# qqaazz0222/DuCoSy-GAN

Hardware: AMD Instinct MI355X
Metric: CycleGAN train-step images/sec at 512x512 bs=8/GPU (higher is better)
Workload: dtype f32 via f16x3 MFMA (power-of-two scaled hi/lo fp16 split, 22 significant bits, three products; f32 accumulation and storage); 1 GPU; full soft-tissue CycleGAN train step: 2x Generator (ResNet-9 + CBAM) + 2x PatchGAN, 9 G loss terms + 2 D losses, 3 Adam steps; img_size=512, per_gpu_batch=8, global_batch=8, residual_blocks=9, input_channels=3, parallelism=dp1

## Files before the change

ducosy-gan_amd/csrc/cbam.hip:

```cpp
#include "common.hpp"

constexpr int SERIAL_UNROLL = 8;

namespace dcs {

__global__ __launch_bounds__(256) void ca_forward_kernel(const float* __restrict__ ymax, const float* __restrict__ sc,
                                                         const float* __restrict__ sh, const float* __restrict__ w1,
                                                         const float* __restrict__ w2, int C, int Cr,
                                                         float* __restrict__ ca) {
    extern __shared__ float sm[];
    float* vmax = sm;
    float* h = sm + C;
    float* h0 = h + Cr;
    const int n = blockIdx.x, tid = threadIdx.x;
    for (int c = tid; c < C; c += blockDim.x) vmax[c] = fmaf(ymax[n * C + c], sc[n * C + c], sh[n * C + c]);
    __syncthreads();
    for (int j = tid; j < Cr; j += blockDim.x) {
        float a = 0.f;
        for (int c = 0; c < C; ++c) a = fmaf(w1[j * C + c], vmax[c], a);
        h[j] = a > 0.f ? a : 0.f;
        h0[j] = 0.f;
    }
    __syncthreads();
    for (int c = tid; c < C; c += blockDim.x) {
// ... 254 lines not shown
        v[k] = reinterpret_cast<const float4*>(y + (p0 + k) * 256)[lane];
        d[k] = reinterpret_cast<const float4*>(dout + (p0 + k) * 256)[lane];
    }
#pragma unroll
    for (int k = 0; k < PX; ++k) {
        float acc = 0.f;
        acc = fmaf(d[k].x, fmaf(v[k].x, s.x, b.x) * a.x, acc);
        acc = fmaf(d[k].y, fmaf(v[k].y, s.y, b.y) * a.y, acc);
        acc = fmaf(d[k].z, fmaf(v[k].z, s.z, b.z) * a.z, acc);
        acc = fmaf(d[k].w, fmaf(v[k].w, s.w, b.w) * a.w, acc);
        acc = wave_sum(acc);
        if (lane == 0) {
            const float g = sa[p0 + k];
            dpre[p0 + k] = acc * g * (1.f - g);
        }
    }
}

template <int PX>
__global__ __launch_bounds__(256) void cb_bwd_dsa_sums_kernel(const float* __restrict__ dout, const float* __restrict__ y,
                                                              const float* __restrict__ sc, const float* __restrict__ sh,
                                                              const float* __restrict__ ca, const float* __restrict__ sa,
                                                              int HW, int nchunk, float* __restrict__ dpre,
                                                              Sum2* __restrict__ p1) {
    __shared__ float4 s_a[256], s_b[256];
    const int n = blockIdx.x, chunk = blockIdx.y, tid = threadIdx.x;
    const int lane = tid & 63, plane = tid >> 6;
    const int p_per = (HW + nchunk - 1) / nchunk;
    const int p0 = chunk * p_per;
    const int pend = min(HW, p0 + p_per);
    const float4 s = reinterpret_cast<const float4*>(sc + (long long)n * 256)[lane];
    const float4 b = reinterpret_cast<const float4*>(sh + (long long)n * 256)[lane];
    const float4 a = reinterpret_cast<const float4*>(ca + (long long)n * 256)[lane];
    float4 A = make_float4(0.f, 0.f, 0.f, 0.f), B = A;
    const long long base = (long long)n * HW;
    for (int p = p0 + plane; p < pend; p += 4 * PX) {
        float4 v[PX], d[PX];
        float gg[PX];
#pragma unroll
        for (int k = 0; k < PX; ++k) {
            const int pk = p + 4 * k < pend ? p + 4 * k : pend - 1;
            v[k] = reinterpret_cast<const float4*>(y + (base + pk) * 256)[lane];
            d[k] = reinterpret_cast<const float4*>(dout + (base + pk) * 256)[lane];
            gg[k] = sa[base + pk];
        }
#pragma unroll
        for (int k = 0; k < PX; ++k) {
            const bool ok = p + 4 * k < pend;
            const float zx = fmaf(v[k].x, s.x, b.x), zy = fmaf(v[k].y, s.y, b.y);
            const float zz = fmaf(v[k].z, s.z, b.z), zw = fmaf(v[k].w, s.w, b.w);
            float acc = 0.f;
            acc = fmaf(d[k].x, zx * a.x, acc);
            acc = fmaf(d[k].y, zy * a.y, acc);
            acc = fmaf(d[k].z, zz * a.z, acc);
            acc = fmaf(d[k].w, zw * a.w, acc);
            acc = wave_sum(acc);
            if (ok) {
                if (lane == 0) dpre[base + p + 4 * k] = acc * gg[k] * (1.f - gg[k]);
                const float g = gg[k];
                const float dx = d[k].x * g, dy_ = d[k].y * g, dz = d[k].z * g, dw = d[k].w * g;
                A.x = fmaf(dx, zx, A.x); A.y = fmaf(dy_, zy, A.y); A.z = fmaf(dz, zz, A.z); A.w = fmaf(dw, zw, A.w);
                B.x += dx; B.y += dy_; B.z += dz; B.w += dw;
            }
        }
    }
    s_a[tid] = A;
    s_b[tid] = B;
    __syncthreads();
    if (plane == 0) {
#pragma unroll
        for (int l = 1; l < 4; ++l) {
            const float4 u = s_a[l * 64 + lane], w = s_b[l * 64 + lane];
            A.x += u.x; A.y += u.y; A.z += u.z; A.w += u.w;
            B.x += w.x; B.y += w.y; B.z += w.z; B.w += w.w;
        }
        Sum2* o = p1 + ((long long)n * nchunk + chunk) * 256 + 4 * lane;
        o[0] = Sum2{A.x, B.x};
        o[1] = Sum2{A.y, B.y};
        o[2] = Sum2{A.z, B.z};
        o[3] = Sum2{A.w, B.w};
    }
}

__global__ void cb_bwd_dsin_kernel(const float* __restrict__ dpre, const float* __restrict__ wsa, int H, int W, int ksa,
                                   long long P, float* __restrict__ dsin) {
    const long long q = (long long)blockIdx.x * blockDim.x + threadIdx.x;
    if (q >= P) return;
    const int HW = H * W;
    const int n = (int)(q / HW);
    const int rem = (int)(q - (long long)n * HW);
    const int qy = rem / W, qx = rem - qy * W;
    const int r = ksa / 2, taps = ksa * ksa;
    float a0 = 0.f, a1 = 0.f;
    for (int ty = 0; ty < ksa; ++ty) {
        int yy = qy - ty + r;
        if (yy < 0 || yy >= H) continue;
        for (int tx = 0; tx < ksa; ++tx) {
            int xx = qx - tx + r;
            if (xx < 0 || xx >= W) continue;
            float d = dpre[(long long)n * HW + yy * W + xx];
            a0 = fmaf(wsa[ty * ksa + tx], d, a0);
            a1 = fmaf(wsa[taps + ty * ksa + tx], d, a1);
        }
    }
    dsin[q * 2 + 0] = a0;
    dsin[q * 2 + 1] = a1;
}

__global__ __launch_bounds__(256) void cb_bwd_dwsa_partial_kernel(const float* __restrict__ dpre,
                                                                  const float* __restrict__ sin_, int H, int W,
                                                                  int ksa, long long P, int nchunk,
                                                                  float* __restrict__ part) {
    __shared__ float red[4];
    const int t = blockIdx.x, chunk = blockIdx.y;
    const int taps = ksa * ksa, r = ksa / 2;
    const int ch = t / taps, tt = t - ch * taps;
    const int ty = tt / ksa, tx = tt - ty * ksa;
    const int per = (int)((P + nchunk - 1) / nchunk);
    const int p0 = chunk * per, p1 = (int)min(P, (long long)p0 + per);
    const int HW = H * W;
    float acc = 0.f;
#pragma unroll 4
    for (int p = p0 + threadIdx.x; p < p1; p += blockDim.x) {
        const int n = p / HW;
        const int rem = p - n * HW;
        const int py = rem / W, px = rem - py * W;
        const int yy = py + ty - r, xx = px + tx - r;
        if (yy >= 0 && yy < H && xx >= 0 && xx < W)
            acc = fmaf(dpre[p], sin_[(n * HW + yy * W + xx) * 2 + ch], acc);
    }
    acc = block_sum_256(acc, red);
    if (threadIdx.x == 0) part[(long long)chunk * gridDim.x + t] = acc;
}

__global__ void cb_bwd_dwsa_final_kernel(const float* __restrict__ part, int nt, int nchunk, float* __restrict__ dwsa) {
    int t = blockIdx.x * blockDim.x + threadIdx.x;
    if (t >= nt) return;
    double s = 0.0;
#pragma unroll SERIAL_UNROLL
    for (int k = 0; k < nchunk; ++k) s += part[(long long)k * nt + t];
    dwsa[t] = (float)s;
}

struct Sum3 {
    float a, b, c;
};

__global__ __launch_bounds__(256) void cb_bwd_sums_kernel(const float* __restrict__ dout, const float* __restrict__ y,
                                                          const float* __restrict__ sc, const float* __restrict__ sh,
                                                          const float* __restrict__ ca, const float* __restrict__ sa,
                                                          const float* __restrict__ dsin,
                                                          const int* __restrict__ sarg, int HW, int C, int nchunk,
                                                          Sum3* __restrict__ parts) {
    const int n = blockIdx.x, chunk = blockIdx.y, tid = threadIdx.x;
    const int p_per = (HW + nchunk - 1) / nchunk;
    const int p0 = chunk * p_per;
    const int p1 = min(HW, p0 + p_per);
    const bool packed = (C <= 256) && (256 % C == 0);
    const int lanes = packed ? 256 / C : 1;
    const int plane = packed ? tid / C : 0;
    __shared__ float s_a[256], s_b[256], s_c[256];
    const float invC = 1.f / (float)C;
    for (int cbase = 0; cbase < C; cbase += (packed ? C : 256)) {
        const int c = packed ? (tid % C) : (cbase + tid);
        float A = 0.f, B = 0.f, Cc = 0.f;
        if (c < C) {
            const long long nc = (long long)n * C + c;
            const float s = sc[nc], b = sh[nc], a = ca[nc];
            for (int p = p0 + plane; p < p1; p += lanes) {
                const long long pp = (long long)n * HW + p;
                const long long o = pp * C + c;
                float z = fmaf(y[o], s, b);
                float dzc = fmaf(dout[o], sa[pp], dsin[pp * 2] * invC);
                if (sarg[pp] == c) dzc += dsin[pp * 2 + 1];
                float dz0 = dzc * a;
                A = fmaf(dzc, z, A);
                B += dz0;
                Cc = fmaf(dz0, z, Cc);
            }
        }
        if (packed) {
            s_a[tid] = A; s_b[tid] = B; s_c[tid] = Cc;
            __syncthreads();
            if (plane == 0) {
                for (int l = 1; l < lanes; ++l) { A += s_a[l * C + c]; B += s_b[l * C + c]; Cc += s_c[l * C + c]; }
                parts[((long long)n * nchunk + chunk) * C + c] = Sum3{A, B, Cc};
            }
            __syncthreads();
        } else if (c < C) {
            parts[((long long)n * nchunk + chunk) * C + c] = Sum3{A, B, Cc};
        }
    }
}

template <bool HALF>
__global__ __launch_bounds__(256) void cb_bwd_sums4_kernel(const float* __restrict__ dout, const float* __restrict__ y,
                                                           const float* __restrict__ sc, const float* __restrict__ sh,
                                                           const float* __restrict__ ca, const float* __restrict__ sa,
                                                           const float* __restrict__ dsin,
                                                           const int* __restrict__ sarg, int HW, int C, int nchunk,
                                                           Sum3* __restrict__ parts, const Sum2* __restrict__ p1) {
    __shared__ float4 s_a[256], s_b[256], s_c[256];
    const int n = blockIdx.x, chunk = blockIdx.y, tid = threadIdx.x;
    const int C4 = C >> 2, lanes = 256 / C4;
    const int c4 = tid % C4, plane = tid / C4;
    const int p_per = (HW + nchunk - 1) / nchunk;
    const int p0 = chunk * p_per;
    const int pend = min(HW, p0 + p_per);
    const int nc = n * C + 4 * c4;
    const float4 s = *reinterpret_cast<const float4*>(sc + nc);
    const float4 b = *reinterpret_cast<const float4*>(sh + nc);
    const float4 a = *reinterpret_cast<const float4*>(ca + nc);
    const float invC = 1.f / (float)C;
    float4 A = make_float4(0.f, 0.f, 0.f, 0.f), B = A, Cc = A;
    for (int p = p0 + plane; p < pend; p += lanes) {
        const long long pp = (long long)n * HW + p;
        const float4 yv = reinterpret_cast<const float4*>(y + pp * C)[c4];
        const float2 ds = reinterpret_cast<const float2*>(dsin)[pp];
        const int am = sarg[pp] - 4 * c4;
        const float d0 = ds.x * invC;
        float z, dzc, dz0;
        if constexpr (HALF) {
#define DCS_SUMS_LANE(X, K)                                   \
        z = fmaf(yv.X, s.X, b.X);                             \
        dzc = d0;                                             \
        if (am == K) dzc += ds.y;                             \
        A.X = fmaf(dzc, z, A.X);                              \
        B.X += dzc;
            DCS_SUMS_LANE(x, 0)
            DCS_SUMS_LANE(y, 1)
            DCS_SUMS_LANE(z, 2)
            DCS_SUMS_LANE(w, 3)
#undef DCS_SUMS_LANE
        } else {
            const float4 dv = reinterpret_cast<const float4*>(dout + pp * C)[c4];
            const float g = sa[pp];
#define DCS_SUMS_LANE(X, K)                                   \
        z = fmaf(yv.X, s.X, b.X);                             \
        dzc = fmaf(dv.X, g, d0);                              \
        if (am == K) dzc += ds.y;                             \
        dz0 = dzc * a.X;                                      \
        A.X = fmaf(dzc, z, A.X);                              \
        B.X += dz0;                                           \
        Cc.X = fmaf(dz0, z, Cc.X);
            DCS_SUMS_LANE(x, 0)
            DCS_SUMS_LANE(y, 1)
            DCS_SUMS_LANE(z, 2)
            DCS_SUMS_LANE(w, 3)
#undef DCS_SUMS_LANE
        }
    }
    s_a[tid] = A; s_b[tid] = B; s_c[tid] = Cc;
    __syncthreads();
    if (plane == 0) {
        for (int l = 1; l < lanes; ++l) {
            const float4 u = s_a[l * C4 + c4], v = s_b[l * C4 + c4], w = s_c[l * C4 + c4];
            A.x += u.x; A.y += u.y; A.z += u.z; A.w += u.w;
            B.x += v.x; B.y += v.y; B.z += v.z; B.w += v.w;
            Cc.x += w.x; Cc.y += w.y; Cc.z += w.z; Cc.w += w.w;
        }
        Sum3* o = parts + ((long long)n * nchunk + chunk) * C + 4 * c4;
        if constexpr (HALF) {
            const Sum2* q = p1 + ((long long)n * nchunk + chunk) * C + 4 * c4;
            const float ax = A.x + q[0].a, ay = A.y + q[1].a, az = A.z + q[2].a, aw = A.w + q[3].a;
            o[0] = Sum3{ax, a.x * (B.x + q[0].b), a.x * ax};
            o[1] = Sum3{ay, a.y * (B.y + q[1].b), a.y * ay};
            o[2] = Sum3{az, a.z * (B.z + q[2].b), a.z * az};
            o[3] = Sum3{aw, a.w * (B.w + q[3].b), a.w * aw};
        } else {
            o[0] = Sum3{A.x, B.x, Cc.x};
            o[1] = Sum3{A.y, B.y, Cc.y};
            o[2] = Sum3{A.z, B.z, Cc.z};
            o[3] = Sum3{A.w, B.w, Cc.w};
        }
    }
}

__global__ __launch_bounds__(256) void cb_bwd_ca_kernel(const Sum3* __restrict__ parts, int nchunk,
                                                        const float* __restrict__ ymax, const float* __restrict__ sc,
                                                        const float* __restrict__ sh, const float* __restrict__ ca,
                                                        const float* __restrict__ w1, const float* __restrict__ w2,
                                                        int HW, int C, int Cr, Sum3* __restrict__ coef,
                                                        float* __restrict__ dwpart) {
    extern __shared__ float sm[];
    float* vmax = sm;
    float* dpc = vmax + C;
    float* hp = dpc + C;
    float* dhm = hp + Cr;
    float* S1 = dhm + Cr;
    float* S2 = S1 + C;
    __shared__ float red[2][4];
    const int tid = threadIdx.x, n = blockIdx.x;
    for (int c = tid; c < C; c += blockDim.x) {
        const long long nc = (long long)n * C + c;
        double A = 0.0, B = 0.0, Cc = 0.0;
#pragma unroll SERIAL_UNROLL
        for (int k = 0; k < nchunk; ++k) {
            Sum3 p = parts[((long long)n * nchunk + k) * C + c];
            A += p.a; B += p.b; Cc += p.c;
        }
        vmax[c] = fmaf(ymax[nc], sc[nc], sh[nc]);
        float g = ca[nc];
        dpc[c] = (float)A * g * (1.f - g);
        S1[c] = (float)B;
        S2[c] = (float)Cc;
    }
    __syncthreads();
    for (int j = 0; j < Cr; ++j) {
        float a = 0.f, b = 0.f;
        for (int c = tid; c < C; c += blockDim.x) {
            a = fmaf(w1[j * C + c], vmax[c], a);
            b = fmaf(w2[c * Cr + j], dpc[c], b);
        }
        a = wave_sum(a);
        b = wave_sum(b);
        if ((tid & 63) == 0) { red[0][tid >> 6] = a; red[1][tid >> 6] = b; }
        __syncthreads();
        if (tid == 0) {
            float hpre = red[0][0] + red[0][1] + red[0][2] + red[0][3];
            float dh = red[1][0] + red[1][1] + red[1][2] + red[1][3];
            hp[j] = hpre;
            dhm[j] = hpre > 0.f ? dh : 0.f;
        }
        __syncthreads();
    }
    float* dw1 = dwpart + (long long)n * 2 * C * Cr;
    float* dw2 = dw1 + (long long)C * Cr;
    const float inv = 1.f / (float)HW;
    for (int c = tid; c < C; c += blockDim.x) {
        float dvm = 0.f;
        for (int j = 0; j < Cr; ++j) {
            dvm = fmaf(w1[j * C + c], dhm[j], dvm);
            dw2[c * Cr + j] = dpc[c] * (hp[j] > 0.f ? hp[j] : 0.f);
            dw1[j * C + c] = dhm[j] * vmax[c];
        }
        coef[(long long)n * C + c] = Sum3{(S1[c] + dvm) * inv, (S2[c] + dvm * vmax[c]) * inv, dvm};
    }
}

__global__ void cb_bwd_dw_reduce_kernel(const float* __restrict__ dwpart, int N, int CCr, float* __restrict__ dw1,
                                        float* __restrict__ dw2) {
    int i = blockIdx.x * blockDim.x + threadIdx.x;
    if (i >= 2 * CCr) return;
    float s = 0.f;
#pragma unroll SERIAL_UNROLL
    for (int n = 0; n < N; ++n) s += dwpart[(long long)n * 2 * CCr + i];
    if (i < CCr) dw1[i] = s;
    else dw2[i - CCr] = s;
}

__global__ void cb_bwd_apply_kernel(const float* __restrict__ dout, const float* __restrict__ y,
                                    const float* __restrict__ sc, const float* __restrict__ sh,
                                    const float* __restrict__ ca, const float* __restrict__ sa,
                                    const float* __restrict__ dsin, const int* __restrict__ sarg,
                                    const int* __restrict__ yarg, const Sum3* __restrict__ coef, int HW, int C,
                                    long long total, float* __restrict__ dy, float* __restrict__ rng) {
    const long long i0 = (long long)blockIdx.x * blockDim.x + threadIdx.x;
    const bool live = i0 < total;
    const long long i = live ? i0 : total - 1;
    const int c = (int)(i % C);
    const long long pp = i / C;
    const int n = (int)(pp / HW);
    const int p = (int)(pp - (long long)n * HW);
    const long long nc = (long long)n * C + c;
    const float s = sc[nc], b = sh[nc];
    const float z = fmaf(y[i], s, b);
    float dzc = fmaf(dout[i], sa[pp], dsin[pp * 2] * (1.f / (float)C));
    if (sarg[pp] == c) dzc += dsin[pp * 2 + 1];
    const Sum3 k = coef[nc];
    float dz = dzc * ca[nc];
    if (yarg[nc] == p) dz += k.c;
    const float v = s * (dz - k.a - z * k.b);
    if (live) dy[i] = v;
    range_note(rng, fabsf(v));
}

__global__ __launch_bounds__(256) void cb_bwd_apply4_kernel(const float* __restrict__ dout, const float* __restrict__ y,
                                                            const float* __restrict__ sc, const float* __restrict__ sh,
                                                            const float* __restrict__ ca, const float* __restrict__ sa,
                                                            const float* __restrict__ dsin, const int* __restrict__ sarg,
                                                            const int* __restrict__ yarg, const Sum3* __restrict__ coef,
                                                            int HW, int C, int total4, float* __restrict__ dy,
                                                            float* __restrict__ rng) {
    const int i40 = blockIdx.x * blockDim.x + threadIdx.x;
    const bool live = i40 < total4;
    const int i4 = live ? i40 : total4 - 1;
    const int C4 = C >> 2;
    const int pp = i4 / C4;
    const int c4 = i4 - pp * C4;
    const int n = pp / HW;
    const int p = pp - n * HW;
    const int nc = n * C + 4 * c4;
    const float4 s = *reinterpret_cast<const float4*>(sc + nc);
    const float4 b = *reinterpret_cast<const float4*>(sh + nc);
    const float4 a = *reinterpret_cast<const float4*>(ca + nc);
    const int4 ya = *reinterpret_cast<const int4*>(yarg + nc);
    const float4 k0 = *reinterpret_cast<const float4*>(reinterpret_cast<const float*>(coef + nc));
    const float4 k1 = *reinterpret_cast<const float4*>(reinterpret_cast<const float*>(coef + nc) + 4);
    const float4 k2 = *reinterpret_cast<const float4*>(reinterpret_cast<const float*>(coef + nc) + 8);
    const float4 yv = reinterpret_cast<const float4*>(y)[i4];
    const float4 dv = reinterpret_cast<const float4*>(dout)[i4];
    const float g = sa[pp];
    const float2 ds = reinterpret_cast<const float2*>(dsin)[pp];
    const int am = sarg[pp] - 4 * c4;
    const float d0 = ds.x * (1.f / (float)C);
    float4 o;
#define DCS_APPLY_LANE(X, K, KA, KB, KC)                      \
    {                                                         \
        const float z = fmaf(yv.X, s.X, b.X);                 \
        float dzc = fmaf(dv.X, g, d0);                        \
        if (am == K) dzc += ds.y;                             \
        float dz = dzc * a.X;                                 \
        if (ya.X == p) dz += KC;                              \
        o.X = s.X * (dz - KA - z * KB);                       \
    }
    DCS_APPLY_LANE(x, 0, k0.x, k0.y, k0.z)
    DCS_APPLY_LANE(y, 1, k0.w, k1.x, k1.y)
    DCS_APPLY_LANE(z, 2, k1.z, k1.w, k2.x)
    DCS_APPLY_LANE(w, 3, k2.y, k2.z, k2.w)
#undef DCS_APPLY_LANE
    if (live) reinterpret_cast<float4*>(dy)[i4] = o;
    range_note(rng, absmax4(o));
}

template <int PX>
__global__ __launch_bounds__(256) void cb_bwd_apply4x_kernel(const float* __restrict__ dout, const float* __restrict__ y,
                                                             const float* __restrict__ sc, const float* __restrict__ sh,
                                                             const float* __restrict__ ca, const float* __restrict__ sa,
                                                             const float* __restrict__ dsin, const int* __restrict__ sarg,
                                                             const int* __restrict__ yarg, const Sum3* __restrict__ coef,
                                                             int HW, int C, float* __restrict__ dy, float* __restrict__ rng) {
    const int C4 = C >> 2;
    const int ppb = 256 / C4;
    const int c4 = threadIdx.x % C4, pl = threadIdx.x / C4;
    const int pp0 = blockIdx.x * ppb * PX;
    const int n = pp0 / HW;
    const int nc = n * C + 4 * c4;
    const float4 s = *reinterpret_cast<const float4*>(sc + nc);
    const float4 b = *reinterpret_cast<const float4*>(sh + nc);
    const float4 a = *reinterpret_cast<const float4*>(ca + nc);
    const int4 ya = *reinterpret_cast<const int4*>(yarg + nc);
    const float4 k0 = *reinterpret_cast<const float4*>(reinterpret_cast<const float*>(coef + nc));
    const float4 k1 = *reinterpret_cast<const float4*>(reinterpret_cast<const float*>(coef + nc) + 4);
    const float4 k2 = *reinterpret_cast<const float4*>(reinterpret_cast<const float*>(coef + nc) + 8);
    const float rC = 1.f / (float)C;
    float m = 0.f;
#pragma unroll
    for (int k = 0; k < PX; ++k) {
        const int pp = pp0 + k * ppb + pl;
        const int p = pp - n * HW;
        const int i4 = pp * C4 + c4;
        const float4 yv = reinterpret_cast<const float4*>(y)[i4];
        const float4 dv = reinterpret_cast<const float4*>(dout)[i4];
        const float g = sa[pp];
        const float2 ds = reinterpret_cast<const float2*>(dsin)[pp];
        const int am = sarg[pp] - 4 * c4;
        const float d0 = ds.x * rC;
        float4 o;
#define DCS_APPLY_LANE(X, K, KA, KB, KC)                      \
    {                                                         \
        const float z = fmaf(yv.X, s.X, b.X);                 \
        float dzc = fmaf(dv.X, g, d0);                        \
        if (am == K) dzc += ds.y;                             \
        float dz = dzc * a.X;                                 \
        if (ya.X == p) dz += KC;                              \
        o.X = s.X * (dz - KA - z * KB);                       \
    }
        DCS_APPLY_LANE(x, 0, k0.x, k0.y, k0.z)
        DCS_APPLY_LANE(y, 1, k0.w, k1.x, k1.y)
        DCS_APPLY_LANE(z, 2, k1.z, k1.w, k2.x)
        DCS_APPLY_LANE(w, 3, k2.y, k2.z, k2.w)
#undef DCS_APPLY_LANE
        reinterpret_cast<float4*>(dy)[i4] = o;
        m = fmaxf(m, absmax4(o));
    }
    range_note(rng, m);
}

static inline int cb_chunks(int N, int HW) {
    int want = (int)cdiv(1024, N);
    int maxc = (int)cdiv(HW, 64);
    int c = want < maxc ? want : maxc;
    return c < 1 ? 1 : c;
}
static inline int sa_wchunks(long long P) {
    long long c = cdiv(P, 4096);
    if (c < 1) c = 1;
    if (c > 64) c = 64;
    return (int)c;
}

struct CbWs {
    float* dpre;
    float* dsin;
    float* wpart;
    Sum3* parts;
    Sum2* p1;
    Sum3* coef;
    float* dwpart;
    size_t total;
};
static CbWs cb_layout(void* base, int N, int H, int W, int C, int Cr, int ksa) {
    CbWs w;
    long long P = (long long)N * H * W;
    size_t off = 0;
    char* b = reinterpret_cast<char*>(base);
    w.dpre = reinterpret_cast<float*>(b + off); off = align_up(off + P * sizeof(float), 256);
    w.dsin = reinterpret_cast<float*>(b + off); off = align_up(off + 2 * P * sizeof(float), 256);
    w.wpart = reinterpret_cast<float*>(b + off); off = align_up(off + (size_t)sa_wchunks(P) * 2 * ksa * ksa * sizeof(float), 256);
    int nch = cb_chunks(N, H * W);
    w.parts = reinterpret_cast<Sum3*>(b + off); off = align_up(off + (size_t)N * nch * C * sizeof(Sum3), 256);
    w.p1 = reinterpret_cast<Sum2*>(b + off); off = align_up(off + (size_t)N * nch * C * sizeof(Sum2), 256);
    w.coef = reinterpret_cast<Sum3*>(b + off); off = align_up(off + (size_t)N * C * sizeof(Sum3), 256);
    w.dwpart = reinterpret_cast<float*>(b + off); off = align_up(off + (size_t)N * 2 * C * Cr * sizeof(float), 256);
    w.total = off;
    return w;
}

}

using namespace dcs;

extern "C" int dcs_cbam_forward(const float* x, const float* y, const float* scale, const float* shift,
                                const float* ymax, const float* w1, const float* w2, const float* wsa, int N, int H,
                                int W, int C, int Cr, int ksa, float* ca, float* sin_, int32_t* sarg, float* sa,
                                float* out, float* rng, void* stream) {
    if (!x || !y || !scale || !shift || !ymax || !w1 || !w2 || !wsa || !ca || !sin_ || !sarg || !sa || !out)
        return fail(DCS_E_INVALID, "cbam_forward: null pointer");
    if (N <= 0 || H <= 0 || W <= 0 || C <= 0 || C % 4 != 0 || Cr <= 0 || ksa <= 0 || (ksa & 1) == 0)
        return fail(DCS_E_INVALID, "cbam_forward: bad dims");
    hipStream_t s = as_stream(stream);
    long long P = (long long)N * H * W;
    hipLaunchKernelGGL(ca_forward_kernel, dim3(N), dim3(256), (size_t)(C + 2 * Cr) * sizeof(float), s, ymax, scale,
                       shift, w1, w2, C, Cr, ca);
    int e = check_launch("ca_forward");
    if (e) return e;
    const int nq = cb_nq(C);
#define DCS_CB16(K, NQ, ...) hipLaunchKernelGGL((K<NQ>), dim3(cb16_blocks(P)), dim3(256), 0, s, __VA_ARGS__)
    if (nq == 4) DCS_CB16(sa_reduce16_kernel, 4, y, scale, shift, ca, H * W, C, P, sin_, sarg);
    else if (nq == 2) DCS_CB16(sa_reduce16_kernel, 2, y, scale, shift, ca, H * W, C, P, sin_, sarg);
    else if (nq == 1) DCS_CB16(sa_reduce16_kernel, 1, y, scale, shift, ca, H * W, C, P, sin_, sarg);
    else hipLaunchKernelGGL(sa_reduce_kernel, dim3((unsigned)cdiv(P, 4)), dim3(256), 0, s, y, scale, shift, ca, H * W, C,
                            P, sin_, sarg);
    e = check_launch("sa_reduce");
    if (e) return e;
    if ((e = range_zero(rng, s))) return e;
    if (nq == 4) DCS_CB16(sa_apply16_kernel, 4, x, y, scale, shift, ca, sin_, wsa, H, W, C, ksa, P, sa, out, rng);
    else if (nq == 2) DCS_CB16(sa_apply16_kernel, 2, x, y, scale, shift, ca, sin_, wsa, H, W, C, ksa, P, sa, out, rng);
    else if (nq == 1) DCS_CB16(sa_apply16_kernel, 1, x, y, scale, shift, ca, sin_, wsa, H, W, C, ksa, P, sa, out, rng);
    else hipLaunchKernelGGL(sa_apply_kernel, dim3((unsigned)cdiv(P, 4)), dim3(256), 0, s, x, y, scale, shift, ca, sin_,
                            wsa, H, W, C, ksa, P, sa, out, rng);
    return check_launch("sa_apply");
}

extern "C" size_t dcs_cbam_backward_workspace_size(int N, int H, int W, int C, int Cr, int ksa) {
    if (N <= 0 || H <= 0 || W <= 0 || C <= 0 || Cr <= 0 || ksa <= 0) return 0;
    return cb_layout(nullptr, N, H, W, C, Cr, ksa).total;
}

extern "C" int dcs_cbam_backward(const float* dout, const float* y, const float* scale, const float* shift,
                                 const float* ymax, const int32_t* yargmax, const float* w1, const float* w2,
                                 const float* wsa, const float* ca, const float* sin_, const int32_t* sarg,
                                 const float* sa, int N, int H, int W, int C, int Cr, int ksa, float* dy, float* dw1,
                                 float* dw2, float* dwsa, void* ws, size_t ws_bytes, float* rng, void* stream) {
    if (!dout || !y || !scale || !shift || !ymax || !yargmax || !w1 || !w2 || !wsa || !ca || !sin_ || !sarg || !sa ||
        !dy || !dw1 || !dw2 || !dwsa || !ws)
        return fail(DCS_E_INVALID, "cbam_backward: null pointer");
    if (N <= 0 || H <= 0 || W <= 0 || C <= 0 || C % 4 != 0 || Cr <= 0 || ksa <= 0)
        return fail(DCS_E_INVALID, "cbam_backward: bad dims");
    if (ws_bytes < dcs_cbam_backward_workspace_size(N, H, W, C, Cr, ksa))
        return fail(DCS_E_WORKSPACE, "cbam_backward: workspace too small");
    if ((long long)N * H * W * 2 >= (1LL << 31))
        return fail(DCS_E_INVALID, "cbam_backward: N*H*W*2 must fit in 31 bits");
    CbWs w = cb_layout(ws, N, H, W, C, Cr, ksa);
    hipStream_t s = as_stream(stream);
    const long long P = (long long)N * H * W;
    const int HW = H * W;
    constexpr int DPX = 4;
    const int nch = cb_chunks(N, HW);
    const bool fused = C == 256;
    if (fused)
        hipLaunchKernelGGL(cb_bwd_dsa_sums_kernel<DPX>, dim3(N, nch), dim3(256), 0, s, dout, y, scale, shift, ca, sa, HW,
                           nch, w.dpre, w.p1);
    else if (C == 256 && HW % DPX == 0)
        hipLaunchKernelGGL(cb_bwd_dsa64x_kernel<DPX>, dim3((unsigned)cdiv(P, 4 * DPX)), dim3(256), 0, s, dout, y, scale,
                           shift, ca, sa, HW, P, w.dpre);
    else
        hipLaunchKernelGGL(cb_bwd_dsa_kernel, dim3((unsigned)cdiv(P, 4)), dim3(256), 0, s, dout, y, scale, shift, ca, sa,
                           HW, C, P, w.dpre);
    int e = check_launch("cb_bwd_dsa");
    if (e) return e;
    hipLaunchKernelGGL(cb_bwd_dsin_kernel, dim3((unsigned)cdiv(P, 256)), dim3(256), 0, s, w.dpre, wsa, H, W, ksa, P,
                       w.dsin);
    if ((e = check_launch("cb_bwd_dsin"))) return e;
    const int nt = 2 * ksa * ksa, nwc = sa_wchunks(P);
    hipLaunchKernelGGL(cb_bwd_dwsa_partial_kernel, dim3(nt, nwc), dim3(256), 0, s, w.dpre, sin_, H, W, ksa, P, nwc,
                       w.wpart);
    if ((e = check_launch("cb_bwd_dwsa_partial"))) return e;
    hipLaunchKernelGGL(cb_bwd_dwsa_final_kernel, dim3((unsigned)cdiv(nt, 128)), dim3(128), 0, s, w.wpart, nt, nwc, dwsa);
    if ((e = check_launch("cb_bwd_dwsa_final"))) return e;
    const bool v4 = (C % 4 == 0) && (C / 4 <= 256) && (256 % (C / 4) == 0);
    if (fused)
        hipLaunchKernelGGL(cb_bwd_sums4_kernel<true>, dim3(N, nch), dim3(256), 0, s, dout, y, scale, shift, ca, sa, w.dsin,
                           sarg, HW, C, nch, w.parts, w.p1);
    else if (v4)
        hipLaunchKernelGGL(cb_bwd_sums4_kernel<false>, dim3(N, nch), dim3(256), 0, s, dout, y, scale, shift, ca, sa, w.dsin,
                           sarg, HW, C, nch, w.parts, nullptr);
    else
        hipLaunchKernelGGL(cb_bwd_sums_kernel, dim3(N, nch), dim3(256), 0, s, dout, y, scale, shift, ca, sa, w.dsin,
                           sarg, HW, C, nch, w.parts);
    if ((e = check_launch("cb_bwd_sums"))) return e;
    hipLaunchKernelGGL(cb_bwd_ca_kernel, dim3(N), dim3(256), (size_t)(4 * C + 2 * Cr) * sizeof(float), s, w.parts, nch,
                       ymax, scale, shift, ca, w1, w2, HW, C, Cr, w.coef, w.dwpart);
    if ((e = check_launch("cb_bwd_ca"))) return e;
    hipLaunchKernelGGL(cb_bwd_dw_reduce_kernel, dim3((unsigned)cdiv(2LL * C * Cr, 256)), dim3(256), 0, s, w.dwpart, N,
                       C * Cr, dw1, dw2);
    if ((e = check_launch("cb_bwd_dw_reduce"))) return e;
    if ((e = range_zero(rng, s))) return e;
    const long long total = P * C;
    const int C4 = C / 4;
    constexpr int APX = 4;
    if (total / 4 < (1LL << 31) && (long long)N * C < (1LL << 31) && C4 <= 256 && 256 % C4 == 0 &&
        HW % (APX * (256 / C4)) == 0) {
        hipLaunchKernelGGL(cb_bwd_apply4x_kernel<APX>, dim3((unsigned)(P / (APX * (256 / C4)))), dim3(256), 0, s, dout,
                           y, scale, shift, ca, sa, w.dsin, sarg, yargmax, w.coef, HW, C, dy, rng);
    } else if (total / 4 < (1LL << 31) && (long long)N * C < (1LL << 31)) {
        const int total4 = (int)(total / 4);
        hipLaunchKernelGGL(cb_bwd_apply4_kernel, dim3((unsigned)cdiv(total4, 256)), dim3(256), 0, s, dout, y, scale,
                           shift, ca, sa, w.dsin, sarg, yargmax, w.coef, HW, C, total4, dy, rng);
    } else {
        hipLaunchKernelGGL(cb_bwd_apply_kernel, dim3((unsigned)cdiv(total, 256)), dim3(256), 0, s, dout, y, scale, shift,
                           ca, sa, w.dsin, sarg, yargmax, w.coef, HW, C, total, dy, rng);
    }
    return check_launch("cb_bwd_apply");
}
#undef DCS_CB16
```

ducosy-gan_amd/csrc/conv.hip:

```cpp
#include "common.hpp"
#include "conv_common.hpp"

namespace dcs {

typedef __bf16 bf16x8 __attribute__((ext_vector_type(8)));

constexpr int MMA_F32 = 0, MMA_BF16 = 1, MMA_BF16X3 = 3, MMA_BF16X6 = 6;
constexpr int MMA_BF16P = 2;
constexpr int MMA_F16X3 = 7;
constexpr int MMA_F16 = 8;

template <int MMA>
constexpr int lde_bf16() { return MMA == MMA_BF16X3 ? 72 : 40; }

typedef unsigned int u32x4v __attribute__((ext_vector_type(4)));
template <int MMA>
__device__ __forceinline__ void split8(const float4& a, const float4& b, bf16x8& hi, bf16x8& lo) {
    const floatx8 f = {a.x, a.y, a.z, a.w, b.x, b.y, b.z, b.w};
    hi = __builtin_convertvector(f, bf16x8);
    if constexpr (MMA == MMA_BF16X3) {
        u32x4v w;
        __builtin_memcpy(&w, &hi, 16);
        floatx8 r;
#pragma unroll
// ... 1789 lines not shown
    for (int p = 0; p < ny; ++p)
        for (int q = 0; q < nx; ++q) {
            const int yp = ay[p], xp = ax[q];
            if (yp >= 1 && yp <= H && xp >= 1 && xp <= W) continue;
            const int ri = yp == 0 ? xp : (yp == Hp - 1 ? Wp + xp : 2 * Wp + 2 * (yp - 1) + (xp == 0 ? 0 : 1));
            for (int q = 0; q < nsplit; ++q) {
                const float4 v = reinterpret_cast<const float4*>(ring)[(((long long)q * N + n) * ringlen + ri) * C4 + c4];
                s.x += v.x; s.y += v.y; s.z += v.z; s.w += v.w;
            }
        }
    *o = s;
}

__global__ void upsample2_grad_kernel(const float* __restrict__ du, float* __restrict__ dx, int N, int H,
                                      int W, int C4) {
    long long idx = (long long)blockIdx.x * blockDim.x + threadIdx.x;
    long long total = (long long)N * H * W * C4;
    if (idx >= total) return;
    int c4 = (int)(idx % C4);
    long long t = idx / C4;
    int j = (int)(t % W); t /= W;
    int i = (int)(t % H);
    int n = (int)(t / H);
    const float4* u = reinterpret_cast<const float4*>(du);
    const long long W2 = 2LL * W;
    long long b = (((long long)n * 2 * H + 2 * i) * W2 + 2 * j) * C4 + c4;
    float4 a0 = u[b], a1 = u[b + C4], a2 = u[b + W2 * C4], a3 = u[b + W2 * C4 + C4];
    reinterpret_cast<float4*>(dx)[idx] =
        make_float4(a0.x + a1.x + a2.x + a3.x, a0.y + a1.y + a2.y + a3.y, a0.z + a1.z + a2.z + a3.z,
                    a0.w + a1.w + a2.w + a3.w);
}

static int validate(const dcs_conv_desc* d, bool rows) {
    if (!d) return fail(DCS_E_INVALID, "null descriptor");
    if (d->N <= 0 || d->Hs <= 0 || d->Ws <= 0 || d->Cs <= 0 || d->Ho <= 0 || d->Wo <= 0 || d->Co <= 0)
        return fail(DCS_E_INVALID, "conv: non-positive dimension");
    if (d->KH <= 0 || d->KW <= 0 || d->KH * d->KW > 64) return fail(DCS_E_INVALID, "conv: bad kernel");
    if (d->up != 1 && d->up != 2) return fail(DCS_E_INVALID, "conv: up must be 1 or 2");
    if (d->stride != 1 && d->stride != 2) return fail(DCS_E_INVALID, "conv: stride must be 1 or 2");
    if (d->parity < 0 || d->parity > 2) return fail(DCS_E_INVALID, "conv: parity must be 0, 1 or 2");
    if (d->parity == 1 && (d->stride != 2 || d->up != 1 || d->pad_mode != DCS_PAD_ZERO))
        return fail(DCS_E_INVALID, "conv: parity rows need stride 2, no upsample, zero pad");
    if (d->parity == 2 && (d->stride != 1 || d->up != 1 || d->pad_mode != DCS_PAD_ZERO || d->KH != 3 ||
                           d->KW != 3 || d->Ho != 2 * d->Hs || d->Wo != 2 * d->Ws))
        return fail(DCS_E_INVALID, "conv: sub-pixel rows describe nearest-x2 + 3x3 zero-pad conv (up=1, Ho=2Hs)");
    if (d->pad_mode == DCS_PAD_REFLECT && (d->pt >= d->Hs * d->up || d->pl >= d->Ws * d->up))
        return fail(DCS_E_INVALID, "conv: reflect pad larger than the input");
    if (d->csplit < 0 || d->csplit > d->Cs) return fail(DCS_E_INVALID, "conv: bad csplit");
    if (d->cw < 0 || d->cw > d->Cs) return fail(DCS_E_INVALID, "conv: bad cw (weight channels)");
    if (d->mma != MMA_F32 && d->mma != MMA_BF16 && d->mma != MMA_BF16X3 && d->mma != MMA_BF16X6 && d->mma != MMA_F16X3 &&
        d->mma != MMA_F16)
        return fail(DCS_E_INVALID, "conv: mma must be DCS_MMA_F32, DCS_MMA_BF16, DCS_MMA_BF16X3, DCS_MMA_BF16X6, DCS_MMA_F16X3 or DCS_MMA_F16");
    if ((d->mma == MMA_F16X3 || d->mma == MMA_F16) && (!d->rng_a || !d->rng_b || d->rng_a_n <= 0 || d->rng_b_n <= 0 ||
                                d->rng_a_n > 1024 || d->rng_b_n > 1024))
        return fail(DCS_E_INVALID, "conv: DCS_MMA_F16X3 / DCS_MMA_F16 need the operand range records rng_a / rng_b (1..1024 partial maxima)");
    if (!d->parity) {
        int Hv = d->Hs * d->up, Wv = d->Ws * d->up;
        (void)Hv; (void)Wv;
    }
    (void)rows;
    return DCS_OK;
}

static bool vec4_ok(const dcs_conv_desc* d, const float* src) {
    const long long extent = (long long)(d->N - 1) * d->s_n + (long long)(d->Hs - 1) * d->s_h +
                             (long long)(d->Ws - 1) * d->s_w + d->Cs;
    return d->Cs == 4 && d->s_c == 1 && d->csplit == 4 && (d->s_w % 4 == 0) && (d->s_h % 4 == 0) &&
           (d->s_n % 4 == 0) && ((reinterpret_cast<uintptr_t>(src) & 15) == 0) && d->s_n >= 0 && d->s_h >= 0 &&
           d->s_w >= 0 && extent * 4 < (long long)OOB_OFF - 64;
}

static bool vec_ok(const dcs_conv_desc* d, const float* src) {
    const long long extent = (long long)(d->N - 1) * d->s_n + (long long)(d->Hs - 1) * d->s_h +
                             (long long)(d->Ws - 1) * d->s_w + d->Cs;
    return (d->Cs % 16 == 0) && d->s_c == 1 && d->csplit == d->Cs &&
           (d->s_w % 4 == 0) && (d->s_h % 4 == 0) && (d->s_n % 4 == 0) &&
           ((reinterpret_cast<uintptr_t>(src) & 15) == 0) && extent * 4 < (long long)OOB_OFF - 64 &&
           d->s_n >= 0 && d->s_h >= 0 && d->s_w >= 0;
}

bool narrow_tiled_ok(const dcs_conv_desc& d, const float* src);
int launch_narrow_rows_tiled(const dcs_conv_desc& d, const float* src, const float* wp, const float* bias,
                             const float* psc, const float* psh, float* out, hipStream_t s);
bool narrow_small_ok(const dcs_conv_desc& d, const float* src);
int launch_narrow_rows_small(const dcs_conv_desc& d, const float* src, const float* wp, const float* bias,
                             const float* psc, const float* psh, float* out, hipStream_t s);
bool narrow_wgrad_tiled_ok(const dcs_conv_desc& d, const float* src);
int narrow_wgrad_tiled_blocks(const dcs_conv_desc& d);
int launch_narrow_wgrad_tiled(const dcs_conv_desc& d, const float* dy, const float* src, const float* psc,
                              const float* psh, float* part, hipStream_t s);

}

using namespace dcs;

extern "C" int dcs_pack_weights_r(const float* w, int Cout, int Cin, int KH, int KW, int kind, int ci_count,
                                  int Kpad, int ncols, int nmajor, float* out, float* rng, void* stream);
namespace {
unsigned pack_blocks(long long total) {
    const long long b = cdiv(total, 256);
    return (unsigned)(b < 1 ? 1 : (b > DCS_RANGE_PARTS ? DCS_RANGE_PARTS : b));
}
}
extern "C" int dcs_pack_weights(const float* w, int Cout, int Cin, int KH, int KW, int kind, int ci_count,
                                int Kpad, int ncols, int nmajor, float* out, void* stream) {
    return dcs_pack_weights_r(w, Cout, Cin, KH, KW, kind, ci_count, Kpad, ncols, nmajor, out, nullptr, stream);
}

namespace {
const char* pack_args_error(const float* w, int Cout, int Cin, int KH, int KW, int kind, int ci_count, int Kpad,
                            int ncols, const float* out) {
    if (!w || !out || Cout <= 0 || Cin <= 0 || KH <= 0 || KW <= 0 || Kpad <= 0 || ncols <= 0 || ci_count <= 0 ||
        (kind != 5 && ci_count > Cin) || (kind == 5 && ci_count < Cin) || kind < 0 ||
        (kind & 7) > 5 || (kind & ~(7 | DCS_PACK_KSLICE)) ||
        ((kind & DCS_PACK_KSLICE) && (((kind & 7) != 0 && (kind & 7) != 1) ||
                                      ((kind & 7) == 0 ? Cin : Cout) % 16 != 0)))
        return "pack_weights: bad arguments";
    if ((kind == 3 || kind == 4) && (KH != 3 || KW != 3)) return "pack_weights: sub-pixel kinds need 3x3";
    return nullptr;
}
}

extern "C" int dcs_pack_weights_r(const float* w, int Cout, int Cin, int KH, int KW, int kind, int ci_count,
                                  int Kpad, int ncols, int nmajor, float* out, float* rng, void* stream) {
    if (const char* err = pack_args_error(w, Cout, Cin, KH, KW, kind, ci_count, Kpad, ncols, out))
        return fail(DCS_E_INVALID, err);
    long long total = (long long)Kpad * ncols;
    if (rng)
        hipLaunchKernelGGL(pack_weights_r_kernel, dim3(pack_blocks(total)), dim3(256), 0, as_stream(stream), w, Cout, Cin,
                           KH, KW, kind, ci_count, Kpad, ncols, nmajor, out, rng);
    else
        hipLaunchKernelGGL(pack_weights_kernel, dim3((unsigned)cdiv(total, 256)), dim3(256), 0, as_stream(stream), w,
                           Cout, Cin, KH, KW, kind, ci_count, Kpad, ncols, nmajor, out);
    return check_launch("pack_weights");
}

namespace dcs {
__global__ __launch_bounds__(256) void pack_split_h3_kernel(const float* __restrict__ wp, long long total, int ldb,
                                                            const float* __restrict__ rng, int rng_n,
                                                            _Float16* __restrict__ out) {
    const float sc = __builtin_ldexpf(1.f, f16x3_exp(rng, rng_n));
    for (long long i = (long long)blockIdx.x * 256 + threadIdx.x; i < total; i += (long long)gridDim.x * 256) {
        const long long r = i / ldb, k = i - r * ldb;
        const float v = wp[i] * sc;
        const _Float16 h = (_Float16)v;
        out[2 * r * ldb + k] = h;
        out[(2 * r + 1) * ldb + k] = (_Float16)(v - (float)h);
    }
}
}

extern "C" int dcs_pack_split_h3(const float* wpack, int rows, int ldb, const float* rng, int rng_n, void* out,
                                 void* stream) {
    if (!wpack || !rng || !out || rows <= 0 || ldb <= 0 || rng_n <= 0) return fail(DCS_E_INVALID, "pack_split_h3: bad arguments");
    const long long total = (long long)rows * ldb;
    const long long blocks = cdiv(total, 256) < 1024 ? cdiv(total, 256) : 1024;
    hipLaunchKernelGGL(pack_split_h3_kernel, dim3((unsigned)blocks), dim3(256), 0, as_stream(stream), wpack, total, ldb,
                       rng, rng_n, reinterpret_cast<_Float16*>(out));
    return check_launch("pack_split_h3");
}

namespace dcs {
namespace {
__device__ __forceinline__ int pack_job_of(const dcs_pack_job* __restrict__ jobs, int njobs, int b, bool second) {
    int lo = 0, hi = njobs - 1;
    while (lo < hi) {
        const int mid = (lo + hi + 1) >> 1;
// ... 806 lines not shown
        const long long total = (long long)d.Co * d.KH * d.KW * d.Cs;
        hipLaunchKernelGGL(wgrad_reduce_kernel, dim3((unsigned)cdiv(total, 256)), dim3(256), 0, s, w, ns, d.Co, d.Cs,
                           d.KH, d.KW, d.Cs, dw);
        return check_launch("conv_wgrad_reduce");
    }
    const bool res = d.Cs == 256 && d.KH == 3 && d.KW == 3 && d.up == 1 && d.stride == 1 && !d.parity &&
                     d.pro_act == DCS_ACT_NONE && d.epi_act == DCS_ACT_NONE;
    const bool v4 = !vec && vec4_ok(dp, x) && d.pro_act == DCS_ACT_NONE && !d.parity;
    const bool dy_small = (long long)d.N * d.Ho * d.Wo * d.Co * 4 < (long long)OOB_OFF - 64;
    if ((d.mma == MMA_F16X3 || d.mma == MMA_F16) && v4 && d.Cs == 4 && !d.parity && dy_small &&
               d.pro_act == DCS_ACT_NONE && (p.BM == 128 || d.Co == 64) && class_geom(d, 0).Mx >= 16) {
        const bool plain = d.pad_mode == DCS_PAD_ZERO && d.up == 1;
        if (d.mma == MMA_F16X3) {
            if (plain) hipLaunchKernelGGL((conv_wgrad_x6_kernel<2, MMA_F16X3, true>), grid, dim3(NT), 0, s, d, dy, x, psc, psh, w, 2 * p.kt_per_split, gn, gm);
            else hipLaunchKernelGGL((conv_wgrad_x6_kernel<0, MMA_F16X3, true>), grid, dim3(NT), 0, s, d, dy, x, psc, psh, w, 2 * p.kt_per_split, gn, gm);
        } else {
            if (plain) hipLaunchKernelGGL((conv_wgrad_x6_kernel<2, MMA_F16, true>), grid, dim3(NT), 0, s, d, dy, x, psc, psh, w, 2 * p.kt_per_split, gn, gm);
            else hipLaunchKernelGGL((conv_wgrad_x6_kernel<0, MMA_F16, true>), grid, dim3(NT), 0, s, d, dy, x, psc, psh, w, 2 * p.kt_per_split, gn, gm);
        }
    } else if (d.mma != MMA_F32 && vec && dy_small && (p.BM == 128 || (d.Co == 64 && (d.mma == MMA_F16X3 || d.mma == MMA_F16))) &&
               d.parity != 1 && class_geom(d, 0).Mx >= 16) {
        const bool plain = d.pro_act == DCS_ACT_NONE && d.pad_mode == DCS_PAD_ZERO && d.up == 1;
        const bool lrelu = d.pro_act == DCS_ACT_LRELU && d.pad_mode == DCS_PAD_ZERO && d.up == 1;
        if (d.mma == MMA_F16X3) {
            if (res) hipLaunchKernelGGL((conv_wgrad_x6_kernel<1, MMA_F16X3>), grid, dim3(NT), 0, s, d, dy, x, psc, psh, w, 2 * p.kt_per_split, gn, gm);
            else if (plain) hipLaunchKernelGGL((conv_wgrad_x6_kernel<2, MMA_F16X3>), grid, dim3(NT), 0, s, d, dy, x, psc, psh, w, 2 * p.kt_per_split, gn, gm);
            else if (lrelu) hipLaunchKernelGGL((conv_wgrad_x6_kernel<3, MMA_F16X3>), grid, dim3(NT), 0, s, d, dy, x, psc, psh, w, 2 * p.kt_per_split, gn, gm);
            else hipLaunchKernelGGL((conv_wgrad_x6_kernel<0, MMA_F16X3>), grid, dim3(NT), 0, s, d, dy, x, psc, psh, w, 2 * p.kt_per_split, gn, gm);
        } else if (d.mma == MMA_F16) {
            if (res) hipLaunchKernelGGL((conv_wgrad_x6_kernel<1, MMA_F16>), grid, dim3(NT), 0, s, d, dy, x, psc, psh, w, 2 * p.kt_per_split, gn, gm);
            else if (plain) hipLaunchKernelGGL((conv_wgrad_x6_kernel<2, MMA_F16>), grid, dim3(NT), 0, s, d, dy, x, psc, psh, w, 2 * p.kt_per_split, gn, gm);
            else if (lrelu) hipLaunchKernelGGL((conv_wgrad_x6_kernel<3, MMA_F16>), grid, dim3(NT), 0, s, d, dy, x, psc, psh, w, 2 * p.kt_per_split, gn, gm);
            else hipLaunchKernelGGL((conv_wgrad_x6_kernel<0, MMA_F16>), grid, dim3(NT), 0, s, d, dy, x, psc, psh, w, 2 * p.kt_per_split, gn, gm);
        } else if (d.mma == MMA_BF16) {
            if (res) hipLaunchKernelGGL((conv_wgrad_x6_kernel<1, MMA_BF16P>), grid, dim3(NT), 0, s, d, dy, x, psc, psh, w, 2 * p.kt_per_split, gn, gm);
            else hipLaunchKernelGGL((conv_wgrad_x6_kernel<0, MMA_BF16P>), grid, dim3(NT), 0, s, d, dy, x, psc, psh, w, 2 * p.kt_per_split, gn, gm);
        } else if (res) hipLaunchKernelGGL((conv_wgrad_x6_kernel<1>), grid, dim3(NT), 0, s, d, dy, x, psc, psh, w, 2 * p.kt_per_split, gn, gm);
        else hipLaunchKernelGGL((conv_wgrad_x6_kernel<0>), grid, dim3(NT), 0, s, d, dy, x, psc, psh, w, 2 * p.kt_per_split, gn, gm);
    } else if (p.BM == 128) {
        if (vec && res) hipLaunchKernelGGL((conv_wgrad_kernel<128, 128, 1, 1>), grid, dim3(NT), 0, s, d, dy, x, x2, psc, psh, w, p.kt_per_split, gn, gm);
        else if (vec) hipLaunchKernelGGL((conv_wgrad_kernel<128, 128, 1, 0>), grid, dim3(NT), 0, s, d, dy, x, x2, psc, psh, w, p.kt_per_split, gn, gm);
        else if (v4) hipLaunchKernelGGL((conv_wgrad_kernel<128, 128, 2, 0>), grid, dim3(NT), 0, s, d, dy, x, x2, psc, psh, w, p.kt_per_split, gn, gm);
        else hipLaunchKernelGGL((conv_wgrad_kernel<128, 128, 0, 0>), grid, dim3(NT), 0, s, d, dy, x, x2, psc, psh, w, p.kt_per_split, gn, gm);
    } else {
        if (vec) hipLaunchKernelGGL((conv_wgrad_kernel<64, 128, 1, 0>), grid, dim3(NT), 0, s, d, dy, x, x2, psc, psh, w, p.kt_per_split, gn, gm);
        else if (v4) hipLaunchKernelGGL((conv_wgrad_kernel<64, 128, 2, 0>), grid, dim3(NT), 0, s, d, dy, x, x2, psc, psh, w, p.kt_per_split, gn, gm);
        else hipLaunchKernelGGL((conv_wgrad_kernel<64, 128, 0, 0>), grid, dim3(NT), 0, s, d, dy, x, x2, psc, psh, w, p.kt_per_split, gn, gm);
    }
    e = check_launch("conv_wgrad");
    if (e) return e;
    if (d.parity == 2) {
        const long long tot9 = (long long)d.Co * d.Cs * 9;
        hipLaunchKernelGGL(wgrad_subpixel_fold_kernel, dim3((unsigned)cdiv(tot9, 256)), dim3(256), 0, s, w, p.nsplit,
                           d.Co, d.Cs, dw);
        return check_launch("wgrad_subpixel_fold");
    }
    long long total = (long long)d.Co * p.Ktot;
    hipLaunchKernelGGL(wgrad_reduce_kernel, dim3((unsigned)cdiv(total, 256)), dim3(256), 0, s, w, p.nsplit, d.Co,
                       d.Cs, d.KH, d.KW, d.cw > 0 ? d.cw : d.Cs, dw);
    return check_launch("conv_wgrad_reduce");
}

extern "C" int dcs_conv_rows_narrow(const dcs_conv_desc* dp, const float* src, const float* src2,
                                    const float* wpack, const float* bias, const float* psc, const float* psh,
                                    float* out, void* stream) {
    int e = validate(dp, true);
    if (e) return e;
    const dcs_conv_desc& d = *dp;
    if (!src || !wpack || !out) return fail(DCS_E_INVALID, "conv_rows_narrow: null pointer");
    if (d.Co > 4) return fail(DCS_E_INVALID, "conv_rows_narrow: Co must be <= 4");
    if (d.ldb < d.Co) return fail(DCS_E_INVALID, "conv_rows_narrow: ldb < Co");
    const int NO = d.Co <= 1 ? 1 : 4;
    const int Krows = d.KH * d.KW * d.Cs;
    size_t lds = (size_t)Krows * NO * sizeof(float);
    if (lds > 64 * 1024) return fail(DCS_E_INVALID, "conv_rows_narrow: weights exceed 64 KiB of LDS");
    long long Mmax = 0;
    const int ncls = d.parity ? 4 : 1;
    for (int z = 0; z < ncls; ++z) {
        ClassGeom g = class_geom(d, z);
        long long M = (long long)g.My * g.Mx * d.N;
        if (M > Mmax) Mmax = M;
    }
    hipStream_t s = as_stream(stream);
    if (narrow_small_ok(d, src)) return launch_narrow_rows_small(d, src, wpack, bias, psc, psh, out, s);
    if (narrow_tiled_ok(d, src)) return launch_narrow_rows_tiled(d, src, wpack, bias, psc, psh, out, s);
    dim3 grid((unsigned)cdiv(Mmax, 256), ncls);
    const bool vec = vec_ok(dp, src);
    if (d.ldb < NO) return fail(DCS_E_INVALID, "conv_rows_narrow: ldb must be >= 4 when Co > 1");
    if (NO == 1) {
        if (vec) hipLaunchKernelGGL((conv_rows_narrow_kernel<1, true>), grid, dim3(256), lds, s, d, src, src2, wpack, bias, psc, psh, out, Krows);
        else hipLaunchKernelGGL((conv_rows_narrow_kernel<1, false>), grid, dim3(256), lds, s, d, src, src2, wpack, bias, psc, psh, out, Krows);
    } else {
        if (vec) hipLaunchKernelGGL((conv_rows_narrow_kernel<4, true>), grid, dim3(256), lds, s, d, src, src2, wpack, bias, psc, psh, out, Krows);
        else hipLaunchKernelGGL((conv_rows_narrow_kernel<4, false>), grid, dim3(256), lds, s, d, src, src2, wpack, bias, psc, psh, out, Krows);
    }
    return check_launch("conv_rows_narrow");
}

namespace {
long long narrow_pix_per_split(const dcs_conv_desc& d, int* nsplit) {
    ClassGeom g = class_geom(d, 0);
    long long P = (long long)g.My * g.Mx * d.N;
    long long Ktot = (long long)g.ntaps * d.Cs;
    long long kb = cdiv(Ktot, 256);
    long long want = cdiv(2048, kb);
    long long ns = want < P ? want : P;
    if (ns < 1) ns = 1;
    if (ns > 4096) ns = 4096;
    long long pps = cdiv(P, ns);
    *nsplit = (int)cdiv(P, pps);
    return pps;
}
}

extern "C" size_t dcs_conv_wgrad_narrow_workspace_size(const dcs_conv_desc* dp) {
    if (!dp) return 0;
    int ns;
    narrow_pix_per_split(*dp, &ns);
    ClassGeom g = class_geom(*dp, 0);
    size_t naive = (size_t)ns * dp->Co * g.ntaps * dp->Cs * sizeof(float);
    size_t tiled = (size_t)narrow_wgrad_tiled_blocks(*dp) * g.ntaps * dp->Cs * sizeof(float);
    return naive > tiled ? naive : tiled;
}

extern "C" int dcs_conv_wgrad_narrow(const dcs_conv_desc* dp, const float* dy, const float* x, const float* x2,
                                     const float* psc, const float* psh, float* dw, void* ws, size_t ws_bytes,
                                     void* stream) {
    int e = validate(dp, false);
    if (e) return e;
    const dcs_conv_desc& d = *dp;
    if (d.parity || d.Co > 4) return fail(DCS_E_INVALID, "conv_wgrad_narrow: forward conv with Co <= 4 expected");
    if (!dy || !x || !dw || !ws) return fail(DCS_E_INVALID, "conv_wgrad_narrow: null pointer");
    if (ws_bytes < dcs_conv_wgrad_narrow_workspace_size(dp)) return fail(DCS_E_WORKSPACE, "conv_wgrad_narrow: workspace too small");
    int ns;
    long long pps = narrow_pix_per_split(d, &ns);
    ClassGeom g = class_geom(d, 0);
    long long Ktot = (long long)g.ntaps * d.Cs;
    dim3 grid((unsigned)cdiv(Ktot, 256), ns);
    hipStream_t s = as_stream(stream);
    float* w = reinterpret_cast<float*>(ws);
    if (narrow_wgrad_tiled_ok(d, x)) {
        e = launch_narrow_wgrad_tiled(d, dy, x, psc, psh, w, s);
        if (e) return e;
        hipLaunchKernelGGL(wgrad_reduce_kernel, dim3((unsigned)cdiv(Ktot, 256)), dim3(256), 0, s, w,
                           narrow_wgrad_tiled_blocks(d), 1, d.Cs, d.KH, d.KW, d.cw > 0 ? d.cw : d.Cs, dw);
        return check_launch("narrow_wgrad_tiled_reduce");
    }
    if (d.Co == 1) hipLaunchKernelGGL((conv_wgrad_narrow_kernel<1, false>), grid, dim3(256), 0, s, d, dy, x, x2, psc, psh, w, pps);
    else if (d.Co == 2) hipLaunchKernelGGL((conv_wgrad_narrow_kernel<2, false>), grid, dim3(256), 0, s, d, dy, x, x2, psc, psh, w, pps);
    else if (d.Co == 3) hipLaunchKernelGGL((conv_wgrad_narrow_kernel<3, false>), grid, dim3(256), 0, s, d, dy, x, x2, psc, psh, w, pps);
    else hipLaunchKernelGGL((conv_wgrad_narrow_kernel<4, false>), grid, dim3(256), 0, s, d, dy, x, x2, psc, psh, w, pps);
    e = check_launch("conv_wgrad_narrow");
    if (e) return e;
    long long total = (long long)d.Co * Ktot;
    hipLaunchKernelGGL(wgrad_reduce_kernel, dim3((unsigned)cdiv(total, 256)), dim3(256), 0, s, w, ns, d.Co, d.Cs,
                       d.KH, d.KW, d.cw > 0 ? d.cw : d.Cs, dw);
    return check_launch("conv_wgrad_narrow_reduce");
}

__global__ void pack_nhwc4_kernel(const float* __restrict__ x, int c1, const float* __restrict__ x2, int c2,
                                  long long HW, long long total, float4* __restrict__ out, float* __restrict__ rng) {
    const long long p = (long long)blockIdx.x * blockDim.x + threadIdx.x;
    float v[4] = {0.f, 0.f, 0.f, 0.f};
    if (p < total) {
        const long long n = p / HW, hw = p - n * HW;
        for (int c = 0; c < c1; ++c) v[c] = x[(n * c1 + c) * HW + hw];
        for (int c = 0; c < c2; ++c) v[c1 + c] = x2[(n * c2 + c) * HW + hw];
        out[p] = make_float4(v[0], v[1], v[2], v[3]);
    }
    range_note(rng, absmax4(make_float4(v[0], v[1], v[2], v[3])));
}

extern "C" int dcs_pack_nhwc4(const float* x, int c1, const float* x2, int c2, int N, int H, int W, float* out,
                              float* rng, void* stream) {
    if (!x || !out || c1 < 1 || c2 < 0 || c1 + c2 > 4 || (c2 > 0 && !x2) || N <= 0 || H <= 0 || W <= 0 ||
        (reinterpret_cast<uintptr_t>(out) & 15))
        return fail(DCS_E_INVALID, "pack_nhwc4: bad arguments");
    if (int e = range_zero(rng, as_stream(stream))) return e;
    const long long HW = (long long)H * W, total = (long long)N * HW;
    hipLaunchKernelGGL(pack_nhwc4_kernel, dim3((unsigned)cdiv(total, 256)), dim3(256), 0, as_stream(stream), x, c1,
                       x2, c2, HW, total, reinterpret_cast<float4*>(out), rng);
    return check_launch("pack_nhwc4");
}

extern "C" int dcs_reflect_fold(const float* dxpad, const float* addend, float* dx, int N, int H, int W, int C,
                                int pad, void* stream) {
    if (!dxpad || !dx || N <= 0 || H <= 0 || W <= 0 || C <= 0 || pad < 0 || pad > 3 || pad >= H || pad >= W)
        return fail(DCS_E_INVALID, "reflect_fold: bad arguments");
    hipStream_t s = as_stream(stream);
    if (C % 4 == 0 && (long long)N * (H + 2 * pad) * (W + 2 * pad) * (C / 4) < (1LL << 31)) {
        long long total = (long long)N * H * W * (C / 4);
        hipLaunchKernelGGL(reflect_fold_kernel, dim3((unsigned)cdiv(total, 256)), dim3(256), 0, s, dxpad, addend, dx,
                           N, H, W, C / 4, pad);
    } else {
        long long total = (long long)N * H * W * C;
        hipLaunchKernelGGL(reflect_fold_scalar_kernel, dim3((unsigned)cdiv(total, 256)), dim3(256), 0, s, dxpad,
                           addend, dx, N, H, W, C, pad);
    }
    return check_launch("reflect_fold");
}

extern "C" size_t dcs_conv_dgrad_reflect_ring_size(const dcs_conv_desc* dp) {
    if (!dp || dp->Ho < 6 || dp->Wo < 6) return 0;
    const int copies = ring_ksplit(*dp) > RG_COPIES ? ring_ksplit(*dp) : RG_COPIES;
    return (size_t)copies * dp->N * (2 * dp->Wo + 2 * (dp->Ho - 2)) * dp->Co * sizeof(float);
}

extern "C" int dcs_conv_dgrad_reflect(const dcs_conv_desc* dp, const float* dy, const float* wpack,
                                      const float* addend, float* dx, float* ring, void* stream) {
    if (!dp || !dy || !wpack || !dx || !ring) return fail(DCS_E_INVALID, "conv_dgrad_reflect: null pointer");
    const dcs_conv_desc& d = *dp;
    if (d.parity || d.stride != 1 || d.up != 1 || d.pad_mode != DCS_PAD_ZERO ||
        d.pt != d.KH - 1 || d.pl != d.KW - 1 || d.pro_act != DCS_ACT_NONE || d.epi_act != DCS_ACT_NONE ||
        d.Ho != d.Hs + 2 || d.Wo != d.Ws + 2 || d.KH != 3 || d.KW != 3 ||
        d.csplit < d.Cs || d.Co % 4 != 0 || d.Ho < 6 || d.Wo < 6)
        return fail(DCS_E_INVALID, "conv_dgrad_reflect: 3x3 stride-1 data gradient onto the pad-1 grid expected "
                                   "(Ho = Hs + 2, pt = pl = 2, zero pad, no activations)");
    if (ring != dx + (long long)d.N * (d.Ho - 2) * (d.Wo - 2) * d.Co)
        return fail(DCS_E_INVALID, "conv_dgrad_reflect: ring must directly follow dx (one allocation)");
    int e = conv_rows_impl(&d, dy, addend, wpack, nullptr, nullptr, nullptr, dx, nullptr, nullptr, stream, 1);
    if (e) return e;
    const int H = d.Ho - 2, W = d.Wo - 2, C4 = d.Co / 4;
    const long long total = (long long)d.N * (2 * W + 2 * (H - 2)) * C4;
    hipLaunchKernelGGL(reflect_ring_fold_kernel, dim3((unsigned)cdiv(total, 256)), dim3(256), 0, as_stream(stream), ring,
                       dx, d.N, H, W, C4, 1);
    return check_launch("reflect_ring_fold");
}

__global__ __launch_bounds__(256) void reflect_ring_fold_ibw_kernel(const float* __restrict__ ring, float* __restrict__ dx,
// ... 103 lines not shown
```

ducosy-gan_amd/csrc/conv_narrow.hip:

```cpp
#include "common.hpp"

namespace dcs {

constexpr int NT_TH = 16, NT_TW = 64, NT_CC = 8, NT_XT = 4;
constexpr int NARROW_TY_UNROLL = 1;
constexpr int NARROW_WAVES = 3;

__device__ __forceinline__ bool nmap(int v, int Hs, int mode, int& s) {
    if (v < 0 || v >= Hs) {
        if (mode == DCS_PAD_ZERO) return false;
        v = v < 0 ? -v : 2 * (Hs - 1) - v;
        v = v < 0 ? 0 : (v >= Hs ? Hs - 1 : v);
    }
    s = v;
    return true;
}

template <int KH, int KW>
__device__ __forceinline__ void stage_halo(const dcs_conv_desc& d, const float* __restrict__ src,
                                           const float* __restrict__ psc, const float* __restrict__ psh,
                                           int n, int oy0, int ox0, int c0, float* lin) {
    constexpr int HH = NT_TH + KH - 1, HW_ = NT_TW + KW - 1;
    const long long so = (long long)n * d.Cs + c0;
    for (int i = threadIdx.x; i < HH * HW_ * 2; i += blockDim.x) {
// ... 131 lines not shown
#pragma unroll
        for (int q = 0; q < IPT; ++q) {
            const int it = threadIdx.x + q * 256;
            if (it < ITEMS) {
                const int t = it / NT_CC, c = it - t * NT_CC;
                part[(long long)blockIdx.x * (KH * KW * d.Cs) + (long long)t * d.Cs + k * NT_CC + c] = acc[k][q];
            }
        }
}

template <int KH, int KW, int NCH>
__global__ __launch_bounds__(256) void narrow_wgrad_win_kernel(const dcs_conv_desc d, const float* __restrict__ dy,
                                                               const float* __restrict__ src,
                                                               const float* __restrict__ psc,
                                                               const float* __restrict__ psh,
                                                               float* __restrict__ part, int tiles_x, int tiles_y) {
    constexpr int HH = NT_TH + KH - 1, HW_ = NT_TW + KW - 1;
    constexpr int ITEMS = KH * NT_CC;
    constexpr int RG = 256 / ITEMS;
    constexpr int RPG = (NT_TH + RG - 1) / RG;
    __shared__ __attribute__((aligned(16))) float lin[HH * HW_ * NT_CC];
    __shared__ float ldy[NT_TH * NT_TW];
    const int rg = threadIdx.x / ITEMS, item = threadIdx.x - (threadIdx.x / ITEMS) * ITEMS;
    const bool live = rg < RG;
    const int ty = item / NT_CC, c = item - (item / NT_CC) * NT_CC;
    float acc[NCH][KW];
#pragma unroll
    for (int k = 0; k < NCH; ++k)
#pragma unroll
        for (int tx = 0; tx < KW; ++tx) acc[k][tx] = 0.f;
    const int ntiles = tiles_x * tiles_y * d.N;
    for (int tile = blockIdx.x; tile < ntiles; tile += gridDim.x) {
        const int n = tile / (tiles_x * tiles_y);
        const int rem = tile - n * tiles_x * tiles_y;
        const int oy0 = (rem / tiles_x) * NT_TH, ox0 = (rem % tiles_x) * NT_TW;
        __syncthreads();
        for (int i = threadIdx.x; i < NT_TH * NT_TW; i += blockDim.x) {
            const int yy = oy0 + i / NT_TW, xx = ox0 + i % NT_TW;
            ldy[i] = (yy < d.Ho && xx < d.Wo) ? dy[((long long)n * d.Ho + yy) * d.Wo + xx] : 0.f;
        }
#pragma unroll
        for (int k = 0; k < NCH; ++k) {
            __syncthreads();
            stage_halo<KH, KW>(d, src, psc, psh, n, oy0, ox0, k * NT_CC, lin);
            __syncthreads();
            if (live) {
                for (int r = 0; r < RPG; ++r) {
                    const int yy = rg * RPG + r;
                    if (yy >= NT_TH) break;
                    const float* row = lin + (yy + ty) * HW_ * NT_CC + c;
                    const float* g = ldy + yy * NT_TW;
                    float w[KW];
#pragma unroll
                    for (int tx = 0; tx < KW - 1; ++tx) w[tx] = row[tx * NT_CC];
#pragma unroll
                    for (int xx = 0; xx < NT_TW; ++xx) {
                        w[(xx + KW - 1) % KW] = row[(xx + KW - 1) * NT_CC];
                        const float gv = g[xx];
#pragma unroll
                        for (int tx = 0; tx < KW; ++tx) acc[k][tx] = fmaf(gv, w[(xx + tx) % KW], acc[k][tx]);
                    }
                }
            }
        }
    }
    float* red = lin;
#pragma unroll
    for (int k = 0; k < NCH; ++k) {
        __syncthreads();
        if (live)
#pragma unroll
            for (int tx = 0; tx < KW; ++tx) red[(rg * ITEMS + item) * KW + tx] = acc[k][tx];
        __syncthreads();
        for (int i = threadIdx.x; i < ITEMS * KW; i += blockDim.x) {
            const int it = i / KW, tx = i - (i / KW) * KW;
            float sum = 0.f;
            for (int q = 0; q < RG; ++q) sum += red[(q * ITEMS + it) * KW + tx];
            const int tyy = it / NT_CC, cc = it - (it / NT_CC) * NT_CC;
            part[(long long)blockIdx.x * (KH * KW * d.Cs) + (long long)(tyy * KW + tx) * d.Cs + k * NT_CC + cc] = sum;
        }
    }
}

template <int KH, int KW, int CPL>
__global__ __launch_bounds__(256) void narrow_rows_small_kernel(const dcs_conv_desc d, const float* __restrict__ src,
                                                                const float* __restrict__ wp,
                                                                const float* __restrict__ bias,
                                                                const float* __restrict__ psc,
                                                                const float* __restrict__ psh,
                                                                float* __restrict__ out) {
    static_assert(CPL % 4 == 0, "float4 channel groups");
    const int lane = threadIdx.x & 63;
    const int c0 = lane * CPL;
    float w[KH * KW][CPL];
#pragma unroll
    for (int t = 0; t < KH * KW; ++t)
#pragma unroll
        for (int j = 0; j < CPL; ++j) w[t][j] = wp[((long long)t * d.Cs + c0 + j) * d.ldb];
    const float b = bias ? bias[0] : 0.f;
    const long long P = (long long)d.N * d.Ho * d.Wo;
    const long long wave = ((long long)blockIdx.x * blockDim.x + threadIdx.x) >> 6;
    const long long nwaves = ((long long)gridDim.x * blockDim.x) >> 6;
    for (long long p = wave; p < P; p += nwaves) {
        const int n = (int)(p / ((long long)d.Ho * d.Wo));
        const int rem = (int)(p - (long long)n * d.Ho * d.Wo);
        const int oy = rem / d.Wo, ox = rem - (rem / d.Wo) * d.Wo;
        float sc[CPL], sh[CPL];
        if (d.pro_act != DCS_ACT_NONE) {
#pragma unroll
            for (int j = 0; j < CPL; ++j) {
                sc[j] = psc[(long long)n * d.Cs + c0 + j];
                sh[j] = psh[(long long)n * d.Cs + c0 + j];
            }
        }
        float acc = 0.f;
#pragma unroll
        for (int ty = 0; ty < KH; ++ty) {
            const int iy = oy * d.stride + ty - d.pt;
            if (iy < 0 || iy >= d.Hs) continue;
#pragma unroll
            for (int tx = 0; tx < KW; ++tx) {
                const int ix = ox * d.stride + tx - d.pl;
                if (ix < 0 || ix >= d.Ws) continue;
                const float* sp = src + n * d.s_n + iy * d.s_h + ix * d.s_w + c0;
#pragma unroll
                for (int j4 = 0; j4 < CPL / 4; ++j4) {
                    const float4 v4 = *reinterpret_cast<const float4*>(sp + 4 * j4);
                    const float v[4] = {v4.x, v4.y, v4.z, v4.w};
#pragma unroll
                    for (int e = 0; e < 4; ++e) {
                        const int j = 4 * j4 + e;
                        const float a = d.pro_act != DCS_ACT_NONE ? act_apply(fmaf(v[e], sc[j], sh[j]), d.pro_act) : v[e];
                        acc = fmaf(a, w[ty * KW + tx][j], acc);
                    }
                }
            }
        }
#pragma unroll
        for (int o = 32; o >= 1; o >>= 1) acc += __shfl_xor(acc, o, 64);
        if (lane == 0) {
            float v = acc + b;
            if (d.epi_act != DCS_ACT_NONE) v = act_apply(v, d.epi_act);
            out[p] = v;
        }
    }
}

bool narrow_small_ok(const dcs_conv_desc& d, const float* src) {
    return !d.parity && d.Co == 1 && d.up == 1 && d.pad_mode == DCS_PAD_ZERO && d.KH == 4 && d.KW == 4 &&
           (d.Cs == 256 || d.Cs == 512) && d.s_c == 1 && d.csplit == d.Cs && d.s_w % 4 == 0 && d.s_h % 4 == 0 &&
           d.s_n % 4 == 0 && (reinterpret_cast<uintptr_t>(src) & 15) == 0 && (long long)d.Ho * d.Wo <= 64 * 64;
}

int launch_narrow_rows_small(const dcs_conv_desc& d, const float* src, const float* wp, const float* bias,
                             const float* psc, const float* psh, float* out, hipStream_t s) {
    const long long P = (long long)d.N * d.Ho * d.Wo;
    long long blocks = cdiv(P, 4);
    if (blocks > 2048) blocks = 2048;
    if (d.Cs == 512)
        hipLaunchKernelGGL((narrow_rows_small_kernel<4, 4, 8>), dim3((unsigned)blocks), dim3(256), 0, s, d, src, wp, bias,
                           psc, psh, out);
    else
        hipLaunchKernelGGL((narrow_rows_small_kernel<4, 4, 4>), dim3((unsigned)blocks), dim3(256), 0, s, d, src, wp, bias,
                           psc, psh, out);
    return check_launch("narrow_rows_small");
}

bool narrow_tiled_ok(const dcs_conv_desc& d, const float* src) {
    return !d.parity && d.Co == 1 && d.up == 1 && d.stride == 1 && d.Cs % NT_CC == 0 && d.s_c == 1 &&
           d.csplit == d.Cs && (d.s_w % 4 == 0) && (d.s_h % 4 == 0) && (d.s_n % 4 == 0) &&
           ((reinterpret_cast<uintptr_t>(src) & 15) == 0) &&
           ((d.KH == 7 && d.KW == 7) || (d.KH == 4 && d.KW == 4));
}

int launch_narrow_rows_tiled(const dcs_conv_desc& d, const float* src, const float* wp, const float* bias,
                             const float* psc, const float* psh, float* out, hipStream_t s) {
    dim3 grid((unsigned)cdiv(d.Wo, NT_TW), (unsigned)cdiv(d.Ho, NT_TH), d.N);
    if (d.KH == 7)
        hipLaunchKernelGGL((narrow_rows_tiled_kernel<7, 7>), grid, dim3(256), 0, s, d, src, wp, bias, psc, psh, out);
    else
        hipLaunchKernelGGL((narrow_rows_tiled_kernel<4, 4>), grid, dim3(256), 0, s, d, src, wp, bias, psc, psh, out);
    return check_launch("narrow_rows_tiled");
}

bool narrow_wgrad_tiled_ok(const dcs_conv_desc& d, const float* src) {
    return narrow_tiled_ok(d, src) && d.KH == 7 && d.Cs == 64;
}

constexpr int NARROW_WGRAD_BLOCKS = 768;
int narrow_wgrad_tiled_blocks(const dcs_conv_desc& d) {
    long long tiles = cdiv(d.Wo, NT_TW) * cdiv(d.Ho, NT_TH) * d.N;
    return (int)(tiles < NARROW_WGRAD_BLOCKS ? tiles : NARROW_WGRAD_BLOCKS);
}

int launch_narrow_wgrad_tiled(const dcs_conv_desc& d, const float* dy, const float* src, const float* psc,
                              const float* psh, float* part, hipStream_t s) {
    const int tx = (int)cdiv(d.Wo, NT_TW), ty = (int)cdiv(d.Ho, NT_TH);
#ifdef DCS_NARROW_WGRAD_ITEMS
    hipLaunchKernelGGL((narrow_wgrad_tiled_kernel<7, 7, 8>), dim3(narrow_wgrad_tiled_blocks(d)), dim3(256), 0, s, d,
                       dy, src, psc, psh, part, tx, ty);
#else
    hipLaunchKernelGGL((narrow_wgrad_win_kernel<7, 7, 8>), dim3(narrow_wgrad_tiled_blocks(d)), dim3(256), 0, s, d,
                       dy, src, psc, psh, part, tx, ty);
#endif
    return check_launch("narrow_wgrad_tiled");
}

__device__ __forceinline__ int pad_preimages(int i, int H, int pad, int mode, int* a) {
    int n = 0;
    a[n++] = i + pad;
    if (mode == DCS_PAD_REFLECT) {
        if (i >= 1 && i <= pad) a[n++] = pad - i;
        if (i >= H - 1 - pad && i <= H - 2) a[n++] = 2 * (H - 1) - i + pad;
    }
    return n;
}

template <int C, int K>
__global__ __launch_bounds__(256) void dgrad_c1_kernel(const float* __restrict__ dy, int N, int H, int W,
                                                       const float* __restrict__ wk, int mode,
                                                       float* __restrict__ dx) {
    constexpr int pad = (K - 1) / 2;
    const long long p = (long long)blockIdx.x * blockDim.x + threadIdx.x;
    if (p >= (long long)N * H * W) return;
    const int n = (int)(p / ((long long)H * W));
    const int rem = (int)(p - (long long)n * H * W);
    const int y = rem / W, x = rem - (rem / W) * W;
    const bool inner = y > pad && y < H - 1 - pad && x > pad && x < W - 1 - pad;
    int ay[3], ax[3], ny = 1, nx = 1;
    if (!inner) {
        ny = pad_preimages(y, H, pad, mode, ay);
        nx = pad_preimages(x, W, pad, mode, ax);
    }
    const float* d = dy + (long long)n * H * W;
    float acc[C];
#pragma unroll
    for (int c = 0; c < C; ++c) acc[c] = 0.f;
#pragma unroll 1
    for (int ty = 0; ty < K; ++ty) {
        float g[K];
        if (inner) {
            const float* b = d + (long long)(y + pad - ty) * W + x + pad;
#pragma unroll
            for (int tx = 0; tx < K; ++tx) g[tx] = b[-tx];
        } else {
#pragma unroll
            for (int tx = 0; tx < K; ++tx) {
                float s = 0.f;
// ... 155 lines not shown
```

ducosy-gan_amd/modules/hip/lib.py:

```python
from __future__ import annotations

import ctypes
import os
from ctypes import POINTER, c_double, c_float, c_int, c_int32, c_int64, c_size_t, c_void_p, c_char_p

PKG_ROOT = os.path.abspath(os.path.join(os.path.dirname(__file__), "..", ".."))
LIB_PATH = os.environ.get("DUCOSY_HIP_LIB", os.path.join(PKG_ROOT, "lib", "libducosy_hip.so"))

DCS_PAD_ZERO, DCS_PAD_REFLECT = 0, 1
ACT_NONE, ACT_AFFINE, ACT_RELU, ACT_LRELU, ACT_TANH = 0, 1, 2, 3, 4
MMA_F32, MMA_BF16, MMA_BF16X3, MMA_BF16X6, MMA_F16X3, MMA_F16 = 0, 1, 3, 6, 7, 8
RANGE_PARTS = 512
KORDER_TAP, KORDER_SLICE, PACK_KSLICE = 0, 1, 8
VOL_F32, VOL_F64, VOL_I16, VOL_U16 = 0, 1, 2, 3
VOL_MAX_RADIUS, VOL_MAX_MEDIAN, VOL_MINMAX_PARTS = 16, 9, 1024
RESIZE_MAX_TAPS = 18
MET_NSTATS, MET_TILE_X, MET_TILE_Y, MET_PAIR_CHUNK = 9, 64, 32, 8192
MET_MSSSIM_TAPS = 11
MET_REGION_NSUMS, MET_REGION_NSSIM = 21, 8
NMODEL_NSTATS = 11


class ConvDesc(ctypes.Structure):
    _fields_ = [
# ... 22 lines not shown
        ("h3_wexp", c_void_p), ("h3_scratch", c_void_p),
        ("b0", c_int32), ("b1", c_int32), ("p0", c_int32), ("p1", c_int32),
    ]


class GLJob(ctypes.Structure):
    _fields_ = [
        ("pred", c_void_p), ("target", c_void_p), ("source", c_void_p), ("add0", c_void_p), ("add1", c_void_p),
        ("grad", c_void_p), ("n_img", c_int32), ("H", c_int32), ("W", c_int32), ("flags", c_int32),
        ("c_l1", c_float), ("c_grad", c_float), ("c_ssim", c_float), ("c_ca", c_float), ("c_mse", c_float),
        ("t_const", c_float), ("c_add0", c_float), ("c_add1", c_float),
    ]


GL_L1, GL_GRAD, GL_SSIM, GL_CA, GL_MSEC = 1, 2, 4, 8, 16

P = c_void_p
DP = POINTER(ConvDesc)

SIGNATURES = {
    "dcs_last_error": (c_char_p, []),
    "dcs_version": (c_int, []),
    "dcs_pack_weights": (c_int, [P, c_int, c_int, c_int, c_int, c_int, c_int, c_int, c_int, c_int, P, P]),
    "dcs_pack_weights_r": (c_int, [P, c_int, c_int, c_int, c_int, c_int, c_int, c_int, c_int, c_int, P, P, P]),
    "dcs_range_parts": (c_int, [P, c_int, c_int64, c_int, P, P, c_int, P, P]),
    "dcs_pack_weights_h3_scratch_size": (c_size_t, []),
    "dcs_pack_weights_h3": (c_int, [P, c_int, c_int, c_int, c_int, P, P, P, P, P]),
    "dcs_conv3_win_ok": (c_int, [DP, c_int]),
    "dcs_conv3_win_in_stats": (c_int, [DP, P, P, P, P, P, P, c_size_t, P, P]),
    "dcs_pack_split_h3": (c_int, [P, c_int, c_int, P, c_int, P, P]),
    "dcs_pack_plan": (c_int, [P, c_int, POINTER(c_int), POINTER(c_int)]),
    "dcs_pack_subpix_h3": (c_int, [P, c_int, c_int, c_int, P, P, P, P, P]),
    "dcs_subpix_win_dgrad_ok": (c_int, [DP]),
    "dcs_subpix_win_dgrad": (c_int, [DP, P, P, P, P, P, P]),
    "dcs_phase_win_dgrad_inbwd_parts_size": (c_size_t, [DP, c_int]),
    "dcs_phase_win_dgrad_inbwd": (c_int, [DP, c_int, P, P, P, P, P, P, P, P, c_int, P, c_size_t, POINTER(c_int), P]),
    "dcs_stride2_win_ok": (c_int, [DP]),
    "dcs_stride2_win_parts_size": (c_size_t, [DP]),
    "dcs_stride2_win": (c_int, [DP, P, P, P, P, P, P, P, P, c_size_t, POINTER(c_int), P]),
    "dcs_subpix_win_ok": (c_int, [DP]),
    "dcs_subpix_win_parts_size": (c_size_t, [DP]),
    "dcs_subpix_win": (c_int, [DP, P, P, P, P, P, P, c_size_t, POINTER(c_int), P]),
    "dcs_pack_batch": (c_int, [P, c_int, c_int, c_int, P]),
    "dcs_stem_fwd_ok": (c_int, [DP]),
    "dcs_stem_fwd_parts_size": (c_size_t, [DP]),
    "dcs_stem_fwd": (c_int, [DP, P, P, P, P, c_size_t, POINTER(c_int), P]),
    "dcs_stem_wgrad_ok": (c_int, [DP]),
    "dcs_stem_wgrad_workspace_size": (c_size_t, [DP]),
    "dcs_stem_wgrad": (c_int, [DP, P, P, P, P, c_size_t, P]),
    "dcs_head_fwd_proj_ok": (c_int, [DP]),
    "dcs_head_fwd_proj": (c_int, [DP, P, P, P, P, P, P, P, P]),
    "dcs_head_wgrad_proj_workspace_size": (c_size_t, [DP]),
    "dcs_head_wgrad_proj": (c_int, [DP, P, P, P, P, P, P, P, c_size_t, P]),
    "dcs_head_dgrad_in_workspace_size": (c_size_t, [c_int, c_int, c_int]),
    "dcs_head_dgrad_in": (c_int, [P, P, c_int, P, c_int, c_int, c_int, P, P, P, c_int, c_int, P, P, c_size_t, P, P]),
    "dcs_conv_dgrad_reflect_win": (c_int, [DP, P, P, P, P, P, P, P, P, P]),
    "dcs_conv_dgrad_reflect_win_inbwd_parts_size": (c_size_t, [DP]),
    "dcs_conv_dgrad_reflect_win_inbwd": (c_int, [DP, P, P, P, P, P, P, P, P, P, P, c_int, P, c_size_t, P, P]),
    "dcs_conv_rows": (c_int, [DP, P, P, P, P, P, P, P, P]),
    "dcs_conv_rows_in_stats_parts_size": (c_size_t, [DP]),
    "dcs_conv_rows_in_stats": (c_int, [DP, P, P, P, P, P, P, P, P, c_size_t, P, P]),
    "dcs_in_stats_finish": (c_int, [P, c_int, c_int, c_int, c_float, P, P, P, P, P]),
    "dcs_conv_dgrad_c1": (c_int, [P, c_int, c_int, c_int, P, c_int, c_int, c_int, c_int, P, P]),
    "dcs_conv_dgrad_to1_workspace_size": (c_size_t, [c_int, c_int, c_int, c_int]),
    "dcs_conv_dgrad_to1": (c_int, [P, c_int, c_int, c_int, c_int, P, c_int, c_int, c_int, c_int, c_int, c_int, c_int,
                                   P, P, c_size_t, P]),
    "dcs_conv_wgrad_workspace_size": (c_size_t, [DP]),
    "dcs_conv_wgrad": (c_int, [DP, P, P, P, P, P, P, P, c_size_t, P]),
    "dcs_conv_dgrad_reflect_ring_size": (c_size_t, [P]),
    "dcs_conv_dgrad_reflect": (c_int, [P, P, P, P, P, P, P]),
    "dcs_reflect_fold": (c_int, [P, P, P, c_int, c_int, c_int, c_int, c_int, P]),
    "dcs_pack_nhwc4": (c_int, [P, c_int, P, c_int, c_int, c_int, c_int, P, P, P]),
    "dcs_upsample2_grad": (c_int, [P, P, c_int, c_int, c_int, c_int, P]),
    "dcs_in_stats_workspace_size": (c_size_t, [c_int, c_int, c_int]),
    "dcs_in_stats": (c_int, [P, c_int, c_int, c_int, c_float, P, P, P, P, P, c_size_t, P]),
    "dcs_in_apply": (c_int, [P, P, P, P, c_int, c_int, c_int, c_int, P, P]),
    "dcs_in_act_backward": (c_int, [P, P, P, P, P, c_int, c_int, c_int, c_int, P, c_size_t, P, P]),
    "dcs_in_act_backward_parts": (c_int, [P, P, P, P, P, c_int, c_int, c_int, c_int, P, c_int, P, c_size_t, P, P]),
    "dcs_conv_rows_narrow": (c_int, [DP, P, P, P, P, P, P, P, P]),
    "dcs_conv_wgrad_narrow_workspace_size": (c_size_t, [DP]),
    "dcs_conv_wgrad_narrow": (c_int, [DP, P, P, P, P, P, P, P, c_size_t, P]),
    "dcs_cbam_forward": (c_int, [P, P, P, P, P, P, P, P, c_int, c_int, c_int, c_int, c_int, c_int,
                                 P, P, P, P, P, P, P]),
    "dcs_cbam_backward_workspace_size": (c_size_t, [c_int, c_int, c_int, c_int, c_int, c_int]),
    "dcs_cbam_backward": (c_int, [P, P, P, P, P, P, P, P, P, P, P, P, P, c_int, c_int, c_int, c_int,
                                  c_int, c_int, P, P, P, P, P, c_size_t, P, P]),
    "dcs_loss_workspace_size": (c_size_t, [c_int, c_int, c_int]),
    "dcs_gen_loss_fused_ws": (c_size_t, [P, c_int]),
    "dcs_gen_loss_fused": (c_int, [P, c_int, c_float, c_float, c_float, c_float, P, P, P, P, c_int, P, P, c_size_t, P]),
    "dcs_multi_add": (c_int, [c_int, P, P, P, P]),
    "dcs_range_arena_register": (c_int, [P, c_size_t]),
    "dcs_range_arena_unregister": (c_int, [P]),
    "dcs_loss_l1": (c_int, [P, P, c_int64, P, P, P, c_size_t, P]),
    "dcs_loss_mse": (c_int, [P, P, c_int64, P, P, P, c_size_t, P]),
    "dcs_loss_mse_const": (c_int, [P, c_float, c_int64, P, P, P, c_size_t, P]),
    "dcs_loss_gradient": (c_int, [P, P, c_int, c_int, c_int, P, P, P, c_size_t, P]),
    "dcs_loss_contrast_attention": (c_int, [P, P, P, c_int, c_int, c_int, c_float, c_float, c_float,
                                            c_int, P, P, P, c_size_t, P]),
    "dcs_loss_contrast_region": (c_int, [P, P, P, c_int, c_int, c_int, c_float, c_float, P, P, P,
                                         c_size_t, P]),
    "dcs_loss_contrast_edge": (c_int, [P, P, c_int, c_int, c_int, P, P, P, c_size_t, P]),
    "dcs_loss_contrast_region_partial": (c_int, [P, P, P, c_int, c_int, c_int, c_float, P, P, c_size_t, P]),
    "dcs_loss_contrast_region_finish": (c_int, [P, c_int, c_int, c_int, c_float, P, c_float, P, P, P, c_size_t, P]),
    "dcs_loss_contrast_edge_partial": (c_int, [P, P, c_int, c_int, c_int, P, P, c_size_t, P]),
    "dcs_loss_contrast_edge_hist": (c_int, [c_int, c_int, c_int, c_int, P, P, P, c_size_t, P]),
    "dcs_loss_contrast_edge_select": (c_int, [c_int, P, P, c_size_t, P]),
    "dcs_loss_contrast_edge_topk": (c_int, [c_int, c_int, c_int, P, P, c_size_t, P]),
    "dcs_loss_contrast_edge_finish": (c_int, [P, c_int, c_int, c_int, P, c_float, P, P, P, c_size_t, P]),
    "dcs_loss_ssim": (c_int, [P, P, c_int, c_int, c_int, c_float, c_int, c_float, c_float, c_float,
                              P, P, P, c_size_t, P]),
    "dcs_adam_step": (c_int, [P, P, P, P, c_int64, c_float, c_float, c_float, c_float, c_float,
                              c_float, P]),
    "dcs_scale_add": (c_int, [P, P, c_float, c_int64, P]),
    "dcs_scale_dev": (c_int, [P, P, P, c_int64, P]),
    "dcs_act_backward": (c_int, [P, P, P, c_int64, c_int, P, P]),
    "dcs_channel_sum_workspace_size": (c_size_t, [c_int64, c_int]),
    "dcs_channel_sum": (c_int, [P, c_int64, c_int, P, P, c_size_t, P]),
    "dcs_hu_transform": (c_int, [P, c_int, P, P, c_int, c_int, c_int, c_float, c_float, c_int, c_float,
                                 P, P, P]),
    "dcs_masks_workspace_size": (c_size_t, [c_int, c_int, c_int]),
    "dcs_anatomical_masks": (c_int, [P, P, c_int, c_int, c_int, P, P, P, c_int, P, P, c_size_t, P]),
    "dcs_vol_gauss1d": (c_int, [P, c_int, P, c_int, c_int, c_int, c_int, c_int, c_int, POINTER(c_double), P]),
    "dcs_vol_median_z": (c_int, [P, P, c_int, c_int, c_int, c_int, P]),
    "dcs_vol_kalman_z": (c_int, [P, P, P, c_int, c_int, c_int, P]),
    "dcs_vol_minmax": (c_int, [P, c_int64, P, P, P]),
    "dcs_vol_unsharp_finish": (c_int, [P, c_int, P, P, P, P, c_int64, c_double, c_double, c_float, P, P]),
    "dcs_vol_finish": (c_int, [P, c_int, P, c_int64, c_float, P, P]),
    "dcs_vol_merge": (c_int, [P, P, P, c_int, P, P, c_int, c_int, c_int, c_float, c_float, c_float, c_float,
                              P, P, P]),
    "dcs_vol_translate_merge": (c_int, [P, c_int, P, P, P, P, c_int, c_int, c_int, c_float, c_float, c_float, c_float,
                                        c_float, c_float, P, P, P, P, P]),
    "dcs_vol_merge_enhance": (c_int, [P, P, P, c_int, P, P, c_int, c_int, c_int, c_float, c_float, P, P]),
    "dcs_vol_translate_enhance": (c_int, [P, c_int, P, P, P, P, c_int, c_int, c_int, c_float, c_float, c_float,
                                          c_float, c_float, c_float, P, P, P, P]),
    "dcs_resize_aa": (c_int, [P, P, P, c_int, c_int, c_int, c_int, c_int, P, P, P, c_int, P, P, P, c_int, P]),
    "dcs_resize_nearest": (c_int, [P, P, c_int, c_int, c_int, c_int, c_int, P]),
    "dcs_met_workspace_size": (c_size_t, [c_int, c_int, c_int]),
    "dcs_met_pair_stats": (c_int, [P, P, c_int, c_int, c_int, POINTER(c_float), P, P, c_size_t, P]),
    "dcs_met_ssim": (c_int, [P, P, c_int, c_int, c_int, POINTER(c_float), c_double, P, P, c_size_t, P]),
    "dcs_met_sobel_ts": (c_int, [P, P, c_int, c_int, c_int, P, P, c_size_t, P]),
    "dcs_met_ed": (c_int, [P, P, c_int, c_int, c_int, P, P, P, c_size_t, P]),
    "dcs_met_sorted_l1": (c_int, [P, P, c_int, c_int, c_int, POINTER(c_float), P, P, c_size_t, P]),
    "dcs_met_normalize": (c_int, [P, c_int64, c_float, c_float, P, P]),
    "dcs_met_msssim_level": (c_int, [P, P, c_int, c_int, c_int, POINTER(c_double), c_double, c_double, P, P, c_size_t,
                                     P]),
    "dcs_met_pool2": (c_int, [P, P, P, P, c_int, c_int, c_int, P]),
    "dcs_met_region_workspace_size": (c_size_t, [c_int, c_int, c_int]),
    "dcs_met_region_sums": (c_int, [P, P, P, c_int, c_int, c_int, POINTER(c_float), P, P, P, c_size_t, P]),
    "dcs_met_region_ssim": (c_int, [P, P, P, c_int, c_int, c_int, c_double, P, P, c_size_t, P]),
    "dcs_lpips_stem": (c_int, [P, c_int, c_int, c_int, c_float, c_float, P, P, P, P]),
    "dcs_lpips_tap_workspace_size": (c_size_t, [c_int, c_int, c_int]),
    "dcs_lpips_tap": (c_int, [P, P, c_int, c_int, c_int, c_int, P, P, P, P, P, c_size_t, P]),
    "dcs_unet_normalize_hu": (c_int, [P, c_int64, c_int, P, P]),
    "dcs_unet_affine_relu_pool": (c_int, [P, P, P, c_int, c_int, c_int, c_int, P, c_int, P, P]),
    "dcs_unet_upsample2_pad": (c_int, [P, P, P, c_int, c_int, c_int, c_int, c_int, c_int, P, c_int, P]),
    "dcs_unet_out_diffmap": (c_int, [P, P, P, P, c_float, c_int64, c_int, c_float, P, P, P, P]),
    "dcs_unet_apply_diffmap": (c_int, [P, c_int64, c_float, P, P, P]),
    "dcs_unet_bn_stats_workspace_size": (c_size_t, [c_int64, c_int]),
    "dcs_unet_bn_stats": (c_int, [P, c_int64, c_int, P, P, c_float, c_float, c_int, P, P, P, P, P, P, P, c_size_t, P]),
    "dcs_unet_bn_relu_backward_workspace_size": (c_size_t, [c_int, c_int, c_int, c_int]),
    "dcs_unet_bn_relu_backward_sums": (c_int, [P, c_int, P, P, P, P, P, P, P, P, c_int, c_int, c_int, c_int, P, P, P, P,
                                               P, c_size_t, P]),
    "dcs_unet_bn_relu_backward_apply": (c_int, [P, c_int, P, P, P, P, P, P, P, P, c_int, c_int, c_int, c_int, P, P, P,
                                                P]),
    "dcs_unet_l1_out_workspace_size": (c_size_t, [c_int64, c_int]),
    "dcs_unet_l1_out": (c_int, [P, P, P, P, P, P, c_int64, c_int, c_float, P, P, P, P, c_size_t, P]),
# ... 65 lines not shown
```

ducosy-gan_amd/modules/hip/ops.py:

```python
from __future__ import annotations

import contextlib
import ctypes
import os
from dataclasses import dataclass
from typing import Optional, Tuple

import torch

from . import lib
from .lib import ACT_AFFINE, ACT_LRELU, ACT_NONE, ACT_RELU, ACT_TANH, DCS_PAD_REFLECT, DCS_PAD_ZERO

IN_EPS = 1e-5

_MMA_NAMES = {"f32": lib.MMA_F32, "bf16": lib.MMA_BF16, "bf16x3": lib.MMA_BF16X3, "bf16x6": lib.MMA_BF16X6,
              "f16x3": lib.MMA_F16X3, "f16": lib.MMA_F16}
_MMA = _MMA_NAMES[os.environ.get("DUCOSY_MMA", "f16x3")]
_STEM = True
_SUBWIN = True
_FUSE_FOLD = True
_WIN = True
_PHASE_F16X3 = frozenset()
_FIXED_F16X3 = frozenset(x for x in os.environ.get("DUCOSY_F16X3_LAYERS", "").split(",") if x)

# ... 365 lines not shown
                     _p(wexp), _stream())
        assert not hasattr(wpack, "_dcs_sp")
        wpack._dcs_h3 = (hi, lo, wexp)
        return wpack

    @property
    def subwin(self) -> bool:
        return _SUBWIN and _h3() and self.subpixel and self.cout % 64 == 0 and self.cin % 16 == 0

    @property
    def s2win(self) -> bool:
        return (_SUBWIN and _h3() and self.stride == 2 and self.k in (3, 4) and self.up == 1 and
                self.pads == (1, 1, 1, 1) and self.pad_mode == DCS_PAD_ZERO and self.cout % 128 == 0 and
                self.cin % 64 == 0)

    def _attach_sp(self, wpack: torch.Tensor, w: torch.Tensor, kind: int = 0) -> torch.Tensor:
        shape = {0: (4 * self.cout, 4 * self.cin), 1: (self.cin, 16 * self.cout), 2: (4 * self.cin, 4 * self.cout),
                 3: (self.cout, 16 * self.cin), 4: (self.cout, 16 * self.cin), 5: (4 * self.cin, 4 * self.cout)}[kind]
        hi = torch.empty(*shape, device=w.device, dtype=torch.float16)
        lo = torch.empty_like(hi)
        wexp = torch.empty(1, device=w.device, dtype=torch.int32)
        scratch = torch.empty(lib.RANGE_PARTS, device=w.device, dtype=torch.float32)
        if _BATCH is not None:
            _BATCH.add(w, h3=2, Cout=self.cout, Cin=self.cin, h3_flip=kind, h3_hi=hi, h3_lo=lo, h3_wexp=wexp,
                       h3_scratch=scratch)
        else:
            lib.call("dcs_pack_subpix_h3", _p(w), self.cout, self.cin, kind, _p(hi), _p(lo), _p(scratch), _p(wexp),
                     _stream())
        assert not hasattr(wpack, "_dcs_h3")
        wpack._dcs_sp = (hi, lo, wexp)
        return wpack

    def _key(self):
        return (self.cin, self.cout, self.k, self.stride, self.pads, self.pad_mode, self.up)

    def pack_fwd(self, w: torch.Tensor, cin_pad: Optional[int] = None) -> torch.Tensor:
        _record_pack(w, "pack_fwd", self, cin_pad)
        return _cached_pack(w, ("fwd", self._key(), cin_pad), lambda: self._pack_fwd(w, cin_pad))

    def pack_dgrad(self, w: torch.Tensor, ci_count: Optional[int] = None) -> torch.Tensor:
        _record_pack(w, "pack_dgrad", self, ci_count)
        return _cached_pack(w, ("dgrad", self._key(), ci_count), lambda: self._pack_dgrad(w, ci_count))

    def _pack_fwd(self, w: torch.Tensor, cin_pad: Optional[int] = None) -> torch.Tensor:
        if cin_pad is not None and cin_pad != self.cin:
            return self._pack(w, 5, cin_pad, self.k * self.k * cin_pad, self.cout)
        if self.subpixel:
            out = self._pack(w, 3, self.cin, 16 * self.cin, self.cout)
            return self._attach_sp(out, w) if self.subwin else out
        K = self.k * self.k * self.cin
        out = self._pack(w, 0, self.cin, K, self.cout)
        if self.s2win:
            return self._attach_sp(out, w, 3 if self.k == 3 else 4)
        return self._attach_h3(out, w, 0) if self.win else out

    @property
    def c1_dgrad(self) -> bool:
        t, l, b, r = self.pads
        return (self.cout == 1 and self.cin in (32, 64) and self.k in (3, 7) and self.stride == 1 and self.up == 1
                and t == l == b == r and 2 * t == self.k - 1)

    def to1_dgrad(self, ci: int) -> bool:
        t, l, b, r = self.pads
        return (ci == 1 and self.cout == 64 and self.up == 1 and (self.k, self.stride) in ((7, 1), (4, 2))
                and (self.pad_mode == DCS_PAD_ZERO or (t == b and l == r)))

    def _pack_dgrad(self, w: torch.Tensor, ci_count: Optional[int] = None) -> torch.Tensor:
        ci = self.cin if ci_count is None else ci_count
        if self.c1_dgrad and ci == self.cin:
            return self._pack(w, 0, self.cin, self.k * self.k * self.cin, 1)
        if self.to1_dgrad(ci):
            return self._pack(w, 2, 1, self.k * self.k * self.cout, 1)
        if self.subpixel and ci > 4:
            out = self._pack(w, 4, ci, 16 * self.cout, ci)
            return self._attach_sp(out, w, 1) if (self.subwin and ci == self.cin and ci % 128 == 0) else out
        kind = 2 if self.stride == 2 else 1
        K = self.k * self.k * self.cout
        out = self._pack(w, kind, ci, K, ci)
        if self.s2win and ci == self.cin:
            return self._attach_sp(out, w, 2 if self.k == 3 else 5)
        return self._attach_h3(out, w, 1) if (self.win and ci == self.cin) else out

    def _pack(self, w, kind, ci_count, K, ncols):
        if kind in (0, 1) and ncols > 4 and self.kslice:
            kind |= lib.PACK_KSLICE
        if ncols <= 4:
            Kpad, cols, nmajor = K, (1 if ncols == 1 else 4), 0
            out = torch.empty(Kpad, cols, device=w.device, dtype=torch.float32)
        else:
            Kpad, cols, nmajor = _round_up(K, 32), _round_up(ncols, _bn_for(ncols)), 1
            out = torch.empty(cols, Kpad, device=w.device, dtype=torch.float32)
        job = dict(Cout=self.cout, Cin=self.cin, KH=self.k, KW=self.k, kind=kind, ci_count=ci_count, Kpad=Kpad,
                   ncols=cols, nmajor=nmajor, out=out)
        if nmajor and _h3():
            rng = torch.empty(lib.RANGE_PARTS, device=w.device, dtype=torch.float32)
            out._dcs_rng = (out._version, None, ACT_NONE, rng)
            planes = None
            if not self.win:
                planes = torch.empty(cols * 2 * Kpad, device=w.device, dtype=torch.float16)
                out._dcs_bh3 = (out._version, planes)
            if _BATCH is not None:
                _BATCH.add(w, rng=rng, planes=planes, **job)
            else:
                lib.call("dcs_pack_weights_r", _p(w), self.cout, self.cin, self.k, self.k, kind, ci_count, Kpad,
                         cols, nmajor, _p(out), _p(rng), _stream())
                if planes is not None:
                    lib.call("dcs_pack_split_h3", _p(out), cols, Kpad, _p(rng), lib.RANGE_PARTS, _p(planes),
                             _stream())
        elif _BATCH is not None:
            _BATCH.add(w, **job)
        else:
            lib.call("dcs_pack_weights", _p(w), self.cout, self.cin, self.k, self.k, kind, ci_count, Kpad,
                     cols, nmajor, _p(out), _stream())
        return out

    def _desc_fwd(self, s: Src, ldb: int, pro_act: int, epi_act: int, rows: bool = True) -> lib.ConvDesc:
        Ho, Wo = self.out_hw(s.H, s.W)
        d = lib.ConvDesc()
        d.N, d.Hs, d.Ws, d.Cs = s.N, s.H, s.W, s.C
        d.s_n, d.s_c, d.s_h, d.s_w = s.strides
        d.csplit = s.C if s.csplit is None else s.csplit
        d.s2_n, d.s2_c, d.s2_h, d.s2_w = s.strides2
        d.up, d.pad_mode = self.up, self.pad_mode
        d.KH = d.KW = self.k
        d.pt, d.pl = self.pads[0], self.pads[1]
        d.stride, d.parity = self.stride, 0
        if self.subpixel and rows:
            d.up, d.parity = 1, 2
        d.Ho, d.Wo, d.Co = Ho, Wo, self.cout
        d.ldb, d.pro_act, d.epi_act = ldb, pro_act, epi_act
        d.mma = _MMA if not _h3() else _fallback()
        d.korder = lib.KORDER_SLICE if (rows and self.kslice and not self.narrow) else lib.KORDER_TAP
        return d

    def forward(self, s: Src, wpack: torch.Tensor, bias: Optional[torch.Tensor] = None,
                pro: Optional[Tuple[torch.Tensor, torch.Tensor, int]] = None,
                epi_act: int = ACT_NONE, pro_max: Optional[torch.Tensor] = None) -> torch.Tensor:
        return self._forward(s, wpack, bias, pro, epi_act, pro_max, False, False)

    def forward_in_stats(self, s: Src, wpack: torch.Tensor, bias: Optional[torch.Tensor] = None,
                         pro: Optional[Tuple[torch.Tensor, torch.Tensor, int]] = None,
                         epi_act: int = ACT_NONE, want_max: bool = False):
        return self._forward(s, wpack, bias, pro, epi_act, None, True, want_max)

    @contextlib.contextmanager
    def _probe(self, npix: int, ci: int):
        e0 = PROBE.begin() if _is_res_geom(self) else None
        yield
        PROBE.end(e0, 2.0 * npix * self.cout * ci * self.k * self.k)

    def _forward(self, s: Src, wpack, bias, pro, epi_act, pro_max, stats: bool, want_max: bool):
        assert s.C == self.cin or (s.C == 4 and self.cin < 4), (s.C, self.cin)
        _check_dev(s.t, s.t2, wpack, bias)
        d = self._desc_fwd(s, wpack.shape[1], pro[2] if pro is not None else ACT_NONE, epi_act)
        nb = 0
        if stats:
            nb = 0 if self.narrow else lib.query("dcs_conv_rows_in_stats_parts_size", ctypes.byref(d))
            if nb == 0:
                out = self._forward(s, wpack, bias, pro, epi_act, None, False, False)
                return out, in_stats(out, want_max)
        Ho, Wo = d.Ho, d.Wo
        dev = s.t.device
        if self.narrow and pro is not None and pro_max is not None and _h3() and s.t2 is None:
            d.mma = _fixed_mma("head")
            if lib.query("dcs_head_fwd_proj_ok", ctypes.byref(d)):
                out = torch.empty(s.N, Ho, Wo, self.cout, device=dev, dtype=torch.float32)
# ... 327 lines not shown


def in_act_backward(da: torch.Tensor, y: torch.Tensor, st: INStats, act: int) -> torch.Tensor:
    N, H, W, C = y.shape
    dy = torch.empty_like(y)
    nb = lib.query("dcs_in_stats_workspace_size", N, H * W, C)
    ws = workspace(nb, y.device)
    lib.call("dcs_in_act_backward", _p(da), _p(y), _p(st.scale), _p(st.shift), _p(dy), N, H * W, C,
             act, _p(ws), ws.numel(), _out_rng(dy), _stream())
    return dy


def head_dgrad_in(dy_out: torch.Tensor, wk: torch.Tensor, y: torch.Tensor, st: INStats, act: int) -> Optional[torch.Tensor]:
    N, H, W, C = y.shape
    if not (_h3() and C == 64 and act == ACT_RELU and H >= 8 and W >= 8 and y.is_contiguous()
            and dy_out.numel() == N * H * W and wk.numel() == 49 * 64):
        return None
    _check_dev(dy_out, wk, y)
    dy = torch.empty_like(y)
    ws = workspace(lib.query("dcs_head_dgrad_in_workspace_size", N, H, W), y.device)
    g = dy_out.contiguous()
    g_rng = range_rec(g.view(N, H, W, 1))
    lib.call("dcs_head_dgrad_in", _p(g), _p(g_rng), g_rng.numel(), _p(wk), N, H, W, _p(y), _p(st.scale), _p(st.shift),
             act, _fixed_mma("head"), _p(dy), _p(ws), ws.numel(), _out_rng(dy), _stream())
    return dy


def in_act_backward_parts(da: torch.Tensor, y: torch.Tensor, st: INStats, act: int, parts: torch.Tensor,
                          nchunk: int) -> torch.Tensor:
    N, H, W, C = y.shape
    dy = torch.empty_like(y)
    ws = workspace(N * C * 8, y.device)
    lib.call("dcs_in_act_backward_parts", _p(da), _p(y), _p(st.scale), _p(st.shift), _p(dy), N, H * W, C, act,
             _p(parts), nchunk, _p(ws), ws.numel(), _out_rng(dy), _stream())
    return dy


def act_backward(da: torch.Tensor, y: torch.Tensor, act: int) -> torch.Tensor:
    out = torch.empty_like(y)
    lib.call("dcs_act_backward", _p(da.contiguous()), _p(y), _p(out), y.numel(), act, _out_rng(out), _stream())
    return out


def channel_sum(x: torch.Tensor, out: Optional[torch.Tensor] = None) -> torch.Tensor:
    C = x.shape[-1]
    Pn = x.numel() // C
    if out is None:
        out = torch.empty(C, device=x.device, dtype=torch.float32)
    assert out.numel() == C and out.is_contiguous()
    ws = workspace(lib.query("dcs_channel_sum_workspace_size", Pn, C), x.device)
    lib.call("dcs_channel_sum", _p(x), Pn, C, _p(out), _p(ws), ws.numel(), _stream())
    return out


def scale_add_(y: torch.Tensor, x: torch.Tensor, a: float = 1.0) -> torch.Tensor:
    assert y.numel() == x.numel() and y.is_contiguous() and x.is_contiguous()
    _drop_rng(y)
    lib.call("dcs_scale_add", _p(y), _p(x), float(a), y.numel(), _stream())
    return y


def scale_dev(x: torch.Tensor, s: torch.Tensor) -> torch.Tensor:
    out = torch.empty_like(x)
    lib.call("dcs_scale_dev", _p(x), _p(s), _p(out), x.numel(), _stream())
    return out


def cbam_forward(x, y, st: INStats, w1, w2, wsa):
    N, H, W, C = y.shape
    Cr = w1.shape[0]
    ksa = wsa.shape[-1]
    dev = y.device
    ca = torch.empty(N, C, device=dev, dtype=torch.float32)
    sin_ = torch.empty(N, H * W, 2, device=dev, dtype=torch.float32)
    sarg = torch.empty(N, H * W, device=dev, dtype=torch.int32)
    sa = torch.empty(N, H * W, device=dev, dtype=torch.float32)
    out = torch.empty_like(x)
    lib.call("dcs_cbam_forward", _p(x), _p(y), _p(st.scale), _p(st.shift), _p(st.xmax), _p(w1),
             _p(w2), _p(wsa), N, H, W, C, Cr, ksa, _p(ca), _p(sin_), _p(sarg), _p(sa), _p(out),
             _out_rng(out), _stream())
    return out, (ca, sin_, sarg, sa)


def cbam_backward(dout, y, st: INStats, w1, w2, wsa, saved, out_dw=(None, None, None)):
    ca, sin_, sarg, sa = saved
    N, H, W, C = y.shape
    Cr = w1.shape[0]
    ksa = wsa.shape[-1]
    dy = torch.empty_like(y)
    dw1 = torch.empty_like(w1) if out_dw[0] is None else out_dw[0]
    dw2 = torch.empty_like(w2) if out_dw[1] is None else out_dw[1]
    dwsa = torch.empty_like(wsa) if out_dw[2] is None else out_dw[2]
    for o, ref in ((dw1, w1), (dw2, w2), (dwsa, wsa)):
        assert o.shape == ref.shape and o.is_contiguous()
    nb = lib.query("dcs_cbam_backward_workspace_size", N, H, W, C, Cr, ksa)
    ws = workspace(nb, y.device)
    lib.call("dcs_cbam_backward", _p(dout), _p(y), _p(st.scale), _p(st.shift), _p(st.xmax),
             _p(st.xargmax), _p(w1), _p(w2), _p(wsa), _p(ca), _p(sin_), _p(sarg), _p(sa), N, H, W,
             C, Cr, ksa, _p(dy), _p(dw1), _p(dw2), _p(dwsa), _p(ws), ws.numel(), _out_rng(dy), _stream())
    return dy, dw1, dw2, dwsa


def _plane_dims(t):
    N, C, H, W = t.shape
    assert C == 1, "losses operate on single-channel planes"
    return N, H, W


def _loss_call(name, pred, args, want_grad):
    _check_dev(pred)
    N, H, W = _plane_dims(pred)
    dev = pred.device
    out = torch.empty(1, device=dev, dtype=torch.float32)
    grad = torch.empty_like(pred) if want_grad else None
    ws = workspace(lib.query("dcs_loss_workspace_size", N, H, W), dev)
    lib.call(name, *args(N, H, W), _p(out), _p(grad), _p(ws), ws.numel(), _stream())
    return out.view(()), grad


def loss_l1(pred, target, want_grad=True):
    p, t = pred.contiguous(), target.contiguous()
    return _loss_call("dcs_loss_l1", p, lambda N, H, W: (_p(p), _p(t), p.numel()), want_grad)


def loss_mse(pred, target, want_grad=True):
    p, t = pred.contiguous(), target.contiguous()
    return _loss_call("dcs_loss_mse", p, lambda N, H, W: (_p(p), _p(t), p.numel()), want_grad)


def loss_mse_const(pred, value: float, want_grad=True):
    p = pred.contiguous()
    return _loss_call("dcs_loss_mse_const", p, lambda N, H, W: (_p(p), float(value), p.numel()),
                      want_grad)


def loss_gradient(pred, target, want_grad=True):
    p, t = pred.contiguous(), target.contiguous()
    return _loss_call("dcs_loss_gradient", p, lambda N, H, W: (_p(p), _p(t), N, H, W), want_grad)


def loss_contrast_attention(pred, target, source, sigma, min_w, max_w, k, want_grad=True):
    p, t, s = pred.contiguous(), target.contiguous(), source.contiguous()
    return _loss_call("dcs_loss_contrast_attention", p,
                      lambda N, H, W: (_p(p), _p(t), _p(s), N, H, W, float(sigma), float(min_w),
                                       float(max_w), int(k)), want_grad)


def loss_contrast_region(pred, target, source, threshold, weight, want_grad=True):
    p, t, s = pred.contiguous(), target.contiguous(), source.contiguous()
    return _loss_call("dcs_loss_contrast_region", p,
                      lambda N, H, W: (_p(p), _p(t), _p(s), N, H, W, float(threshold),
                                       float(weight)), want_grad)


def loss_contrast_edge(pred, target, want_grad=True):
    p, t = pred.contiguous(), target.contiguous()
    return _loss_call("dcs_loss_contrast_edge", p, lambda N, H, W: (_p(p), _p(t), N, H, W),
                      want_grad)


def loss_contrast_region_global(pred, target, source, threshold, weight, allreduce, grad_scale, want_grad=True):
    p, t, s = pred.contiguous(), target.contiguous(), source.contiguous()
    _check_dev(p, t, s)
    N, H, W = _plane_dims(p)
    dev = p.device
    ws = workspace(lib.query("dcs_loss_workspace_size", N, H, W), dev)
# ... 158 lines not shown
```

include/ducosy_hip.h:

```cpp
#ifndef DUCOSY_HIP_H
#define DUCOSY_HIP_H

#include <stddef.h>
#include <stdint.h>

#ifdef __cplusplus
extern "C" {
#endif

#define DCS_OK 0
#define DCS_E_INVALID 1001
#define DCS_E_WORKSPACE 1002

#define DCS_PAD_ZERO 0
#define DCS_PAD_REFLECT 1

#define DCS_ACT_NONE 0
#define DCS_ACT_AFFINE 1
#define DCS_ACT_RELU 2
#define DCS_ACT_LRELU 3
#define DCS_ACT_TANH 4

typedef struct dcs_conv_desc {
    int32_t N;
// ... 121 lines not shown
size_t dcs_conv_dgrad_to1_workspace_size(int N, int Hy, int Wy, int K);
int dcs_conv_dgrad_to1(const float* dy, int N, int Hy, int Wy, int C, const float* wk, int K, int stride, int pt,
                       int pl, int pad_mode, int H, int W, float* dx, void* ws, size_t ws_bytes, void* stream);

int dcs_pack_nhwc4(const float* x, int c1, const float* x2, int c2, int N, int H, int W, float* out,
                   float* rng,
                   void* stream);

size_t dcs_conv_dgrad_reflect_ring_size(const dcs_conv_desc* d);
int dcs_conv_dgrad_reflect(const dcs_conv_desc* d, const float* dy, const float* wpack, const float* addend,
                           float* dx, float* ring, void* stream);
int dcs_reflect_fold(const float* dxpad, const float* addend, float* dx, int N, int H, int W, int C,
                     int pad, void* stream);

int dcs_upsample2_grad(const float* dup, float* dx, int N, int H, int W, int C, void* stream);


size_t dcs_in_stats_workspace_size(int N, int HW, int C);
int dcs_in_stats(const float* x, int N, int HW, int C, float eps, float* scale, float* shift,
                 float* xmax, int32_t* xargmax, void* ws, size_t ws_bytes, void* stream);

int dcs_in_stats_finish(const void* parts, int N, int C, int nchunk, float eps, float* scale, float* shift,
                        float* xmax, int32_t* xargmax, void* stream);

int dcs_in_apply(const float* x, const float* scale, const float* shift, float* out, int N, int HW,
                 int C, int act, float* rng,
                 void* stream);

int dcs_in_act_backward(const float* da, const float* y, const float* scale, const float* shift,
                        float* dy, int N, int HW, int C, int act, void* ws, size_t ws_bytes,
                        float* rng,
                        void* stream);
int dcs_in_act_backward_parts(const float* da, const float* y, const float* scale, const float* shift, float* dy,
                              int N, int HW, int C, int act, const void* parts, int nchunk, void* ws,
                              size_t ws_bytes, float* rng, void* stream);

int dcs_conv_rows_narrow(const dcs_conv_desc* d, const float* src, const float* src2,
                         const float* wpack, const float* bias, const float* pro_scale,
                         const float* pro_shift, float* out, void* stream);
int dcs_head_fwd_proj_ok(const dcs_conv_desc* d);
int dcs_head_fwd_proj(const dcs_conv_desc* d, const float* src, const float* wpack, const float* bias,
                      const float* pro_scale, const float* pro_shift, const float* xmax, float* out, void* stream);
size_t dcs_head_wgrad_proj_workspace_size(const dcs_conv_desc* d);
int dcs_head_wgrad_proj(const dcs_conv_desc* d, const float* dy, const float* src, const float* pro_scale,
                        const float* pro_shift, const float* xmax, float* dw, void* ws, size_t ws_bytes,
                        void* stream);
size_t dcs_head_dgrad_in_workspace_size(int N, int H, int W);
int dcs_head_dgrad_in(const float* dy_out, const float* dy_rng, int dy_rng_n, const float* wk, int N, int H, int W,
                      const float* y, const float* scale, const float* shift, int act, int mma, float* dy, void* ws,
                      size_t ws_bytes, float* rng, void* stream);
int dcs_stem_fwd_ok(const dcs_conv_desc* d);
size_t dcs_stem_fwd_parts_size(const dcs_conv_desc* d);
int dcs_stem_fwd(const dcs_conv_desc* d, const float* src, const float* wpack, float* out, void* parts,
                 size_t parts_bytes, int* nchunk, void* stream);
int dcs_stem_wgrad_ok(const dcs_conv_desc* d);
size_t dcs_stem_wgrad_workspace_size(const dcs_conv_desc* d);
int dcs_stem_wgrad(const dcs_conv_desc* d, const float* dy, const float* src, float* dw, void* ws, size_t ws_bytes,
                   void* stream);
int dcs_pack_split_h3(const float* wpack, int rows, int ldb, const float* rng, int rng_n, void* out, void* stream);
typedef struct dcs_pack_job {
    const float* w;
    int32_t Cout, Cin, KH, KW, kind, ci_count, Kpad, ncols, nmajor, h3, h3_flip, h3_ncols;
    float* out;
    float* rng;
    void* planes;
    void* h3_hi;
    void* h3_lo;
    int32_t* h3_wexp;
    float* h3_scratch;
    int32_t b0, b1, p0, p1;
} dcs_pack_job;
int dcs_pack_plan(dcs_pack_job* jobs, int njobs, int* g1, int* g2);
int dcs_pack_batch(const dcs_pack_job* jobs_dev, int njobs, int g1, int g2, void* stream);
size_t dcs_conv_wgrad_narrow_workspace_size(const dcs_conv_desc* d);
int dcs_conv_wgrad_narrow(const dcs_conv_desc* d, const float* dy, const float* x, const float* x2,
                          const float* pro_scale, const float* pro_shift, float* dw, void* ws,
                          size_t ws_bytes, void* stream);

int dcs_cbam_forward(const float* x, const float* y, const float* scale, const float* shift,
                     const float* ymax, const float* w1, const float* w2, const float* wsa,
                     int N, int H, int W, int C, int Cr, int ksa,
                     float* ca, float* sin_, int32_t* sarg, float* sa, float* out, float* rng,
                     void* stream);
size_t dcs_cbam_backward_workspace_size(int N, int H, int W, int C, int Cr, int ksa);
int dcs_cbam_backward(const float* dout, const float* y, const float* scale, const float* shift,
                      const float* ymax, const int32_t* yargmax, const float* w1, const float* w2,
                      const float* wsa, const float* ca, const float* sin_, const int32_t* sarg,
                      const float* sa, int N, int H, int W, int C, int Cr, int ksa, float* dy,
                      float* dw1, float* dw2, float* dwsa, void* ws, size_t ws_bytes, float* rng,
                      void* stream);

int dcs_loss_contrast_region_partial(const float* pred, const float* target, const float* source, int N, int H,
                                     int W, float threshold, double* red, void* ws, size_t ws_bytes, void* stream);
int dcs_loss_contrast_region_finish(const float* pred, int N, int H, int W, float weight, const double* red,
                                    float grad_scale, float* out, float* grad, void* ws, size_t ws_bytes,
                                    void* stream);
int dcs_loss_contrast_edge_partial(const float* pred, const float* target, int N, int H, int W, double* red,
                                   void* ws, size_t ws_bytes, void* stream);
int dcs_loss_contrast_edge_hist(int N, int H, int W, int pass, const double* red, uint32_t* hist, void* ws,
                                size_t ws_bytes, void* stream);
int dcs_loss_contrast_edge_select(int pass, const uint32_t* hist, void* ws, size_t ws_bytes, void* stream);
int dcs_loss_contrast_edge_topk(int N, int H, int W, double* red, void* ws, size_t ws_bytes, void* stream);
int dcs_loss_contrast_edge_finish(const float* pred, int N, int H, int W, const double* red, float grad_scale,
                                  float* out, float* grad, void* ws, size_t ws_bytes, void* stream);

size_t dcs_loss_workspace_size(int N, int H, int W);
int dcs_loss_l1(const float* pred, const float* target, int64_t n, float* out, float* grad,
                void* ws, size_t ws_bytes, void* stream);
int dcs_loss_mse(const float* pred, const float* target, int64_t n, float* out, float* grad,
                 void* ws, size_t ws_bytes, void* stream);
int dcs_loss_mse_const(const float* pred, float target, int64_t n, float* out, float* grad,
                       void* ws, size_t ws_bytes, void* stream);
int dcs_loss_gradient(const float* pred, const float* target, int N, int H, int W, float* out,
                      float* grad, void* ws, size_t ws_bytes, void* stream);
int dcs_loss_contrast_attention(const float* pred, const float* target, const float* source, int N,
                                int H, int W, float sigma, float min_w, float max_w, int k,
                                float* out, float* grad, void* ws, size_t ws_bytes, void* stream);
int dcs_loss_contrast_region(const float* pred, const float* target, const float* source, int N,
                             int H, int W, float threshold, float weight, float* out, float* grad,
                             void* ws, size_t ws_bytes, void* stream);
int dcs_loss_contrast_edge(const float* pred, const float* target, int N, int H, int W, float* out,
                           float* grad, void* ws, size_t ws_bytes, void* stream);
int dcs_loss_ssim(const float* X, const float* Y, int N, int H, int W, float data_range,
                  int win, float sigma, float k1, float k2, float* out, float* grad, void* ws,
                  size_t ws_bytes, void* stream);

int dcs_adam_step(float* p, const float* g, float* m, float* v, int64_t n, float lr, float beta1,
                  float beta2, float eps, float bias_c1, float bias_c2, void* stream);


int dcs_hu_transform(const void* raw, int raw_dtype, const float* slope, const float* intercept, int N,
                     int H, int W, float hu_min, float hu_max, int soft, float sigma, float* hu,
                     float* img, void* stream);

size_t dcs_masks_workspace_size(int N, int H, int W);
int dcs_anatomical_masks(const float* hu, const uint8_t* lung_in, int N, int H, int W, const float* thresholds,
                         const int32_t* iparams, const int32_t* chan, int nout, float* out, void* ws,
                         size_t ws_bytes, void* stream);

#define DCS_VOL_F32 0
#define DCS_VOL_F64 1
#define DCS_VOL_I16 2
#define DCS_VOL_U16 3
#define DCS_VOL_MAX_RADIUS 16
#define DCS_VOL_MAX_MEDIAN 9
#define DCS_VOL_MINMAX_PARTS 1024

int dcs_vol_gauss1d(const void* in, int in_dtype, void* out, int out_dtype, int D, int H, int W, int axis,
                    int radius, const double* weights, void* stream);
int dcs_vol_median_z(const float* in, float* out, int D, int H, int W, int k, void* stream);
int dcs_vol_kalman_z(const float* in, const double* gain, double* out, int D, int H, int W, void* stream);
int dcs_vol_minmax(const float* x, int64_t n, float* out, float* ws, void* stream);
int dcs_vol_unsharp_finish(const void* sm, int sm_dtype, const double* blur_sm, const double* blur_og,
                           const float* original, const float* minmax, int64_t n, double one_minus_amount,
                           double amount, float hu_threshold, int16_t* out, void* stream);
int dcs_vol_finish(const void* sm, int sm_dtype, const float* original, int64_t n, float hu_threshold,
                   int16_t* out, void* stream);
int dcs_vol_merge(const void* raw, const void* soft, const void* lung, int stored_dtype, const float* slope,
                  const float* intercept, int D, int H, int W, float soft_lo, float soft_hi, float lung_lo,
                  float lung_hi, void* out, float* out_f32, void* stream);
int dcs_vol_merge_enhance(const void* raw, const void* soft, const void* lung, int stored_dtype, const float* slope,
                          const float* intercept, int D, int H, int W, float threshold, float min_hu,
                          float* out_f32, void* stream);

#define DCS_RESIZE_MAX_TAPS 18

// ... 102 lines not shown
```

Before: 39.11 img/s.

## Tile CBAM spatial-attention backward, parallelize channel-attention backward, strip narrow convs

Replaces the per-pixel dsin kernel and the strided dwsa partial-sum kernel with one shared-memory tiled kernel. It computes both dsin and per-tile weight-gradient partials and folds them with a templated wave shuffle reduction. The channel-attention backward kernel moves to 1024 threads, splits chunk summation across sub-lanes, and removes per-j block barriers. Narrow Co=1 4x4 conv forward and weight-gradient paths are rewritten as strip kernels, and a standalone SA backward entry point is added. The cost is more code, restriction to ksa 3/5/7, and more partials for the final reduction.

```diff
diff --git a/ducosy-gan_amd/csrc/cbam.hip b/ducosy-gan_amd/csrc/cbam.hip
--- a/ducosy-gan_amd/csrc/cbam.hip
+++ b/ducosy-gan_amd/csrc/cbam.hip
@@ -360,64 +360,119 @@
     }
 }
 
-__global__ void cb_bwd_dsin_kernel(const float* __restrict__ dpre, const float* __restrict__ wsa, int H, int W, int ksa,
-                                   long long P, float* __restrict__ dsin) {
-    const long long q = (long long)blockIdx.x * blockDim.x + threadIdx.x;
-    if (q >= P) return;
-    const int HW = H * W;
-    const int n = (int)(q / HW);
-    const int rem = (int)(q - (long long)n * HW);
-    const int qy = rem / W, qx = rem - qy * W;
-    const int r = ksa / 2, taps = ksa * ksa;
-    float a0 = 0.f, a1 = 0.f;
-    for (int ty = 0; ty < ksa; ++ty) {
-        int yy = qy - ty + r;
-        if (yy < 0 || yy >= H) continue;
-        for (int tx = 0; tx < ksa; ++tx) {
-            int xx = qx - tx + r;
-            if (xx < 0 || xx >= W) continue;
-            float d = dpre[(long long)n * HW + yy * W + xx];
-            a0 = fmaf(wsa[ty * ksa + tx], d, a0);
-            a1 = fmaf(wsa[taps + ty * ksa + tx], d, a1);
-        }
-    }
-    dsin[q * 2 + 0] = a0;
-    dsin[q * 2 + 1] = a1;
-}
-
-__global__ __launch_bounds__(256) void cb_bwd_dwsa_partial_kernel(const float* __restrict__ dpre,
-                                                                  const float* __restrict__ sin_, int H, int W,
-                                                                  int ksa, long long P, int nchunk,
-                                                                  float* __restrict__ part) {
-    __shared__ float red[4];
-    const int t = blockIdx.x, chunk = blockIdx.y;
-    const int taps = ksa * ksa, r = ksa / 2;
-    const int ch = t / taps, tt = t - ch * taps;
-    const int ty = tt / ksa, tx = tt - ty * ksa;
-    const int per = (int)((P + nchunk - 1) / nchunk);
-    const int p0 = chunk * per, p1 = (int)min(P, (long long)p0 + per);
-    const int HW = H * W;
-    float acc = 0.f;
-#pragma unroll 4
-    for (int p = p0 + threadIdx.x; p < p1; p += blockDim.x) {
-        const int n = p / HW;
-        const int rem = p - n * HW;
-        const int py = rem / W, px = rem - py * W;
-        const int yy = py + ty - r, xx = px + tx - r;
-        if (yy >= 0 && yy < H && xx >= 0 && xx < W)
-            acc = fmaf(dpre[p], sin_[(n * HW + yy * W + xx) * 2 + ch], acc);
-    }
-    acc = block_sum_256(acc, red);
-    if (threadIdx.x == 0) part[(long long)chunk * gridDim.x + t] = acc;
-}
-
-__global__ void cb_bwd_dwsa_final_kernel(const float* __restrict__ part, int nt, int nchunk, float* __restrict__ dwsa) {
-    int t = blockIdx.x * blockDim.x + threadIdx.x;
-    if (t >= nt) return;
+template <int NV, int O>
+struct WaveFold {
+    static constexpr int NH = (NV + 1) / 2;
+    static constexpr int live() {
+        if constexpr (O > 1) return WaveFold<NH, O / 2>::live();
+        else return NH;
+    }
+    static __device__ __forceinline__ void run(float* v, int lane) {
+        const bool hi = (lane & O) != 0;
+#pragma unroll
+        for (int i = 0; i < NH; ++i) {
+            const float a = v[i], b = i + NH < NV ? v[i + NH] : 0.f;
+            v[i] = (hi ? b : a) + __shfl_xor(hi ? a : b, O, 64);
+        }
+        if constexpr (O > 1) WaveFold<NH, O / 2>::run(v, lane);
+    }
+    static __device__ __forceinline__ int index(int lane, int s) {
+        if constexpr (O > 1) s = WaveFold<NH, O / 2>::index(lane, s);
+        else if (s >= NH) return -1;
+        if (s < 0 || !(lane & O)) return s;
+        return s + NH < NV ? s + NH : -1;
+    }
+};
+
+constexpr int SAT_H = 16, SAT_W = 64, SAT_PX = 4;
+static inline int sa_tiles(int N, int H, int W) { return N * (int)cdiv(H, SAT_H) * (int)cdiv(W, SAT_W); }
+
+template <int KSA>
+__global__ __launch_bounds__(256) void cb_bwd_sa_tile_kernel(const float* __restrict__ dpre,
+                                                             const float* __restrict__ sin_,
+                                                             const float* __restrict__ wsa, int H, int W,
+                                                             float* __restrict__ dsin, float* __restrict__ part) {
+    constexpr int R = KSA / 2, TAPS = KSA * KSA, NT = 2 * TAPS;
+    constexpr int LH = SAT_H + 2 * R, LW = SAT_W + 2 * R, WIN = SAT_PX + 2 * R;
+    static_assert(NT <= 128, "at most two values per lane after the fold");
+    __shared__ float s_d[LH][LW];
+    __shared__ float2 s_s[LH][LW];
+    __shared__ float s_red[4][NT];
+    const int tid = threadIdx.x, lane = tid & 63, wv = tid >> 6;
+    const int n = blockIdx.z, y0 = blockIdx.y * SAT_H, x0 = blockIdx.x * SAT_W;
+    const int base = n * H * W;
+    for (int i = tid; i < LH * LW; i += 256) {
+        const int ly = i / LW, lx = i - ly * LW;
+        const int yy = y0 + ly - R, xx = x0 + lx - R;
+        const bool in = yy >= 0 && yy < H && xx >= 0 && xx < W;
+        const int p = in ? base + yy * W + xx : base;
+        const float d = dpre[p];
+        const float2 v = reinterpret_cast<const float2*>(sin_)[p];
+        s_d[ly][lx] = in ? d : 0.f;
+        s_s[ly][lx] = in ? v : make_float2(0.f, 0.f);
+    }
+    __syncthreads();
+    const int lx = lane, ry = wv * SAT_PX;
+    {
+        float win[WIN][KSA];
+#pragma unroll
+        for (int j = 0; j < WIN; ++j)
+#pragma unroll
+            for (int c = 0; c < KSA; ++c) win[j][c] = s_d[ry + j][lx + c];
+#pragma unroll
+        for (int k = 0; k < SAT_PX; ++k) {
+            float a0 = 0.f, a1 = 0.f;
+#pragma unroll
+            for (int ty = 0; ty < KSA; ++ty)
+#pragma unroll
+                for (int tx = 0; tx < KSA; ++tx) {
+                    const float d = win[k + 2 * R - ty][2 * R - tx];
+                    a0 = fmaf(wsa[ty * KSA + tx], d, a0);
+                    a1 = fmaf(wsa[TAPS + ty * KSA + tx], d, a1);
+                }
+            const int qy = y0 + ry + k, qx = x0 + lx;
+            if (qy < H && qx < W) reinterpret_cast<float2*>(dsin)[base + qy * W + qx] = make_float2(a0, a1);
+        }
+    }
+    float acc[NT];
+#pragma unroll
+    for (int t = 0; t < NT; ++t) acc[t] = 0.f;
+    float d[SAT_PX];
+#pragma unroll
+    for (int k = 0; k < SAT_PX; ++k) d[k] = s_d[ry + k + R][lx + R];
+#pragma unroll
+    for (int tx = 0; tx < KSA; ++tx) {
+        float2 col[WIN];
+#pragma unroll
+        for (int j = 0; j < WIN; ++j) col[j] = s_s[ry + j][lx + tx];
+#pragma unroll
+        for (int ty = 0; ty < KSA; ++ty)
+#pragma unroll
+            for (int k = 0; k < SAT_PX; ++k) {
+                acc[ty * KSA + tx] = fmaf(d[k], col[k + ty].x, acc[ty * KSA + tx]);
+                acc[TAPS + ty * KSA + tx] = fmaf(d[k], col[k + ty].y, acc[TAPS + ty * KSA + tx]);
+            }
+    }
+    WaveFold<NT, 32>::run(acc, lane);
+#pragma unroll
+    for (int j = 0; j < WaveFold<NT, 32>::live(); ++j) {
+        const int t = WaveFold<NT, 32>::index(lane, j);
+        if (t >= 0) s_red[wv][t] = acc[j];
+    }
+    __syncthreads();
+    if (tid < NT) {
+        const int tile = (blockIdx.z * gridDim.y + blockIdx.y) * gridDim.x + blockIdx.x;
+        part[(long long)tile * NT + tid] = ((s_red[0][tid] + s_red[1][tid]) + s_red[2][tid]) + s_red[3][tid];
+    }
+}
+
+__global__ __launch_bounds__(64) void cb_bwd_dwsa_final_kernel(const float* __restrict__ part, int nt, int ntiles,
+                                                               float* __restrict__ dwsa) {
+    const int t = blockIdx.x, lane = threadIdx.x;
     double s = 0.0;
-#pragma unroll SERIAL_UNROLL
-    for (int k = 0; k < nchunk; ++k) s += part[(long long)k * nt + t];
-    dwsa[t] = (float)s;
+    for (int k = lane; k < ntiles; k += 64) s += part[(long long)k * nt + t];
+    s = wave_sum_d(s);
+    if (lane == 0) dwsa[t] = (float)s;
 }
 
 struct Sum3 {
@@ -554,12 +609,13 @@
     }
 }
 
-__global__ __launch_bounds__(256) void cb_bwd_ca_kernel(const Sum3* __restrict__ parts, int nchunk,
-                                                        const float* __restrict__ ymax, const float* __restrict__ sc,
-                                                        const float* __restrict__ sh, const float* __restrict__ ca,
-                                                        const float* __restrict__ w1, const float* __restrict__ w2,
-                                                        int HW, int C, int Cr, Sum3* __restrict__ coef,
-                                                        float* __restrict__ dwpart) {
+constexpr int CA_SUB = 4, CA_THREADS = 1024;
+__global__ __launch_bounds__(CA_THREADS) void cb_bwd_ca_kernel(const Sum3* __restrict__ parts, int nchunk,
+                                                               const float* __restrict__ ymax, const float* __restrict__ sc,
+                                                               const float* __restrict__ sh, const float* __restrict__ ca,
+                                                               const float* __restrict__ w1, const float* __restrict__ w2,
+                                                               int HW, int C, int Cr, Sum3* __restrict__ coef,
+                                                               float* __restrict__ dwpart) {
     extern __shared__ float sm[];
     float* vmax = sm;
     float* dpc = vmax + C;
@@ -567,51 +623,60 @@
     float* dhm = hp + Cr;
     float* S1 = dhm + Cr;
     float* S2 = S1 + C;
-    __shared__ float red[2][4];
-    const int tid = threadIdx.x, n = blockIdx.x;
-    for (int c = tid; c < C; c += blockDim.x) {
+    const int tid = threadIdx.x, n = blockIdx.x, lane = tid & 63;
+    for (int i = tid; i < CA_SUB * C; i += CA_THREADS) {
+        const int c = i / CA_SUB, sub = i % CA_SUB;
         const long long nc = (long long)n * C + c;
+        const float vm = fmaf(ymax[nc], sc[nc], sh[nc]), g = ca[nc];
         double A = 0.0, B = 0.0, Cc = 0.0;
 #pragma unroll SERIAL_UNROLL
-        for (int k = 0; k < nchunk; ++k) {
+        for (int k = sub; k < nchunk; k += CA_SUB) {
             Sum3 p = parts[((long long)n * nchunk + k) * C + c];
             A += p.a; B += p.b; Cc += p.c;
         }
-        vmax[c] = fmaf(ymax[nc], sc[nc], sh[nc]);
-        float g = ca[nc];
-        dpc[c] = (float)A * g * (1.f - g);
-        S1[c] = (float)B;
-        S2[c] = (float)Cc;
+#pragma unroll
+        for (int o = 1; o < CA_SUB; o <<= 1) {
+            A += __shfl_xor(A, o, 64); B += __shfl_xor(B, o, 64); Cc += __shfl_xor(Cc, o, 64);
+        }
+        if (sub == 0) {
+            vmax[c] = vm;
+            dpc[c] = (float)A * g * (1.f - g);
+            S1[c] = (float)B;
+            S2[c] = (float)Cc;
+        }
     }
     __syncthreads();
-    for (int j = 0; j < Cr; ++j) {
-        float a = 0.f, b = 0.f;
-        for (int c = tid; c < C; c += blockDim.x) {
-            a = fmaf(w1[j * C + c], vmax[c], a);
-            b = fmaf(w2[c * Cr + j], dpc[c], b);
-        }
-        a = wave_sum(a);
-        b = wave_sum(b);
-        if ((tid & 63) == 0) { red[0][tid >> 6] = a; red[1][tid >> 6] = b; }
-        __syncthreads();
-        if (tid == 0) {
-            float hpre = red[0][0] + red[0][1] + red[0][2] + red[0][3];
-            float dh = red[1][0] + red[1][1] + red[1][2] + red[1][3];
+    for (int j = tid >> 6; j < Cr; j += CA_THREADS / 64) {
+        float a[4], b[4];
+#pragma unroll
+        for (int w = 0; w < 4; ++w) {
+            a[w] = 0.f; b[w] = 0.f;
+            for (int c = 64 * w + lane; c < C; c += 256) {
+                a[w] = fmaf(w1[j * C + c], vmax[c], a[w]);
+                b[w] = fmaf(w2[c * Cr + j], dpc[c], b[w]);
+            }
+            a[w] = wave_sum(a[w]);
+            b[w] = wave_sum(b[w]);
+        }
+        if (lane == 0) {
+            const float hpre = a[0] + a[1] + a[2] + a[3];
+            const float dh = b[0] + b[1] + b[2] + b[3];
             hp[j] = hpre;
             dhm[j] = hpre > 0.f ? dh : 0.f;
         }
-        __syncthreads();
-    }
+    }
+    __syncthreads();
     float* dw1 = dwpart + (long long)n * 2 * C * Cr;
     float* dw2 = dw1 + (long long)C * Cr;
+    for (int i = tid; i < C * Cr; i += CA_THREADS) {
+        const int j1 = i / C, c1 = i - j1 * C, c2 = i / Cr, j2 = i - c2 * Cr;
+        dw1[i] = dhm[j1] * vmax[c1];
+        dw2[i] = dpc[c2] * (hp[j2] > 0.f ? hp[j2] : 0.f);
+    }
     const float inv = 1.f / (float)HW;
-    for (int c = tid; c < C; c += blockDim.x) {
+    for (int c = tid; c < C; c += CA_THREADS) {
         float dvm = 0.f;
-        for (int j = 0; j < Cr; ++j) {
-            dvm = fmaf(w1[j * C + c], dhm[j], dvm);
-            dw2[c * Cr + j] = dpc[c] * (hp[j] > 0.f ? hp[j] : 0.f);
-            dw1[j * C + c] = dhm[j] * vmax[c];
-        }
+        for (int j = 0; j < Cr; ++j) dvm = fmaf(w1[j * C + c], dhm[j], dvm);
         coef[(long long)n * C + c] = Sum3{(S1[c] + dvm) * inv, (S2[c] + dvm * vmax[c]) * inv, dvm};
     }
 }
@@ -761,12 +826,6 @@
     int c = want < maxc ? want : maxc;
     return c < 1 ? 1 : c;
 }
-static inline int sa_wchunks(long long P) {
-    long long c = cdiv(P, 4096);
-    if (c < 1) c = 1;
-    if (c > 64) c = 64;
-    return (int)c;
-}
 
 struct CbWs {
     float* dpre;
@@ -785,7 +844,7 @@
     char* b = reinterpret_cast<char*>(base);
     w.dpre = reinterpret_cast<float*>(b + off); off = align_up(off + P * sizeof(float), 256);
     w.dsin = reinterpret_cast<float*>(b + off); off = align_up(off + 2 * P * sizeof(float), 256);
-    w.wpart = reinterpret_cast<float*>(b + off); off = align_up(off + (size_t)sa_wchunks(P) * 2 * ksa * ksa * sizeof(float), 256);
+    w.wpart = reinterpret_cast<float*>(b + off); off = align_up(off + (size_t)sa_tiles(N, H, W) * 2 * ksa * ksa * sizeof(float), 256);
     int nch = cb_chunks(N, H * W);
     w.parts = reinterpret_cast<Sum3*>(b + off); off = align_up(off + (size_t)N * nch * C * sizeof(Sum3), 256);
     w.p1 = reinterpret_cast<Sum2*>(b + off); off = align_up(off + (size_t)N * nch * C * sizeof(Sum2), 256);
@@ -793,6 +852,22 @@
     w.dwpart = reinterpret_cast<float*>(b + off); off = align_up(off + (size_t)N * 2 * C * Cr * sizeof(float), 256);
     w.total = off;
     return w;
+}
+
+static int sa_backward_launch(const float* dpre, const float* sin_, const float* wsa, int N, int H, int W, int ksa,
+                              float* dsin, float* wpart, float* dwsa, hipStream_t s) {
+    const int nt = 2 * ksa * ksa;
+    const dim3 tiles((unsigned)cdiv(W, SAT_W), (unsigned)cdiv(H, SAT_H), N);
+#define DCS_SA_TILE(K) hipLaunchKernelGGL(cb_bwd_sa_tile_kernel<K>, tiles, dim3(256), 0, s, dpre, sin_, wsa, H, W, dsin, wpart)
+    if (ksa == 7) DCS_SA_TILE(7);
+    else if (ksa == 5) DCS_SA_TILE(5);
+    else if (ksa == 3) DCS_SA_TILE(3);
+    else return fail(DCS_E_INVALID, "cbam_backward: the spatial-attention kernel must be 3, 5 or 7 wide");
+#undef DCS_SA_TILE
+    int e = check_launch("cb_bwd_sa_tile");
+    if (e) return e;
+    hipLaunchKernelGGL(cb_bwd_dwsa_final_kernel, dim3(nt), dim3(64), 0, s, wpart, nt, sa_tiles(N, H, W), dwsa);
+    return check_launch("cb_bwd_dwsa_final");
 }
 
 }
@@ -831,6 +906,25 @@
     return check_launch("sa_apply");
 }
 
+extern "C" size_t dcs_cbam_sa_backward_workspace_size(int N, int H, int W, int ksa) {
+    if (N <= 0 || H <= 0 || W <= 0 || ksa <= 0) return 0;
+    return (size_t)sa_tiles(N, H, W) * 2 * ksa * ksa * sizeof(float);
+}
+
+extern "C" int dcs_cbam_sa_backward(const float* dpre, const float* sin_, const float* wsa, int N, int H, int W,
+                                    int ksa, float* dsin, float* dwsa, void* ws, size_t ws_bytes, void* stream) {
+    if (!dpre || !sin_ || !wsa || !dsin || !dwsa || !ws) return fail(DCS_E_INVALID, "cbam_sa_backward: null pointer");
+    if (N <= 0 || H <= 0 || W <= 0) return fail(DCS_E_INVALID, "cbam_sa_backward: bad dims");
+    if (ksa != 3 && ksa != 5 && ksa != 7)
+        return fail(DCS_E_INVALID, "cbam_sa_backward: the spatial-attention kernel must be 3, 5 or 7 wide");
+    if ((long long)N * H * W * 2 >= (1LL << 31))
+        return fail(DCS_E_INVALID, "cbam_sa_backward: N*H*W*2 must fit in 31 bits");
+    if (ws_bytes < dcs_cbam_sa_backward_workspace_size(N, H, W, ksa))
+        return fail(DCS_E_WORKSPACE, "cbam_sa_backward: workspace too small");
+    return sa_backward_launch(dpre, sin_, wsa, N, H, W, ksa, dsin, reinterpret_cast<float*>(ws), dwsa,
+                              as_stream(stream));
+}
+
 extern "C" size_t dcs_cbam_backward_workspace_size(int N, int H, int W, int C, int Cr, int ksa) {
     if (N <= 0 || H <= 0 || W <= 0 || C <= 0 || Cr <= 0 || ksa <= 0) return 0;
     return cb_layout(nullptr, N, H, W, C, Cr, ksa).total;
@@ -846,6 +940,8 @@
         return fail(DCS_E_INVALID, "cbam_backward: null pointer");
     if (N <= 0 || H <= 0 || W <= 0 || C <= 0 || C % 4 != 0 || Cr <= 0 || ksa <= 0)
         return fail(DCS_E_INVALID, "cbam_backward: bad dims");
+    if (ksa != 3 && ksa != 5 && ksa != 7)
+        return fail(DCS_E_INVALID, "cbam_backward: the spatial-attention kernel must be 3, 5 or 7 wide");
     if (ws_bytes < dcs_cbam_backward_workspace_size(N, H, W, C, Cr, ksa))
         return fail(DCS_E_WORKSPACE, "cbam_backward: workspace too small");
     if ((long long)N * H * W * 2 >= (1LL << 31))
@@ -868,15 +964,7 @@
                            HW, C, P, w.dpre);
     int e = check_launch("cb_bwd_dsa");
     if (e) return e;
-    hipLaunchKernelGGL(cb_bwd_dsin_kernel, dim3((unsigned)cdiv(P, 256)), dim3(256), 0, s, w.dpre, wsa, H, W, ksa, P,
-                       w.dsin);
-    if ((e = check_launch("cb_bwd_dsin"))) return e;
-    const int nt = 2 * ksa * ksa, nwc = sa_wchunks(P);
-    hipLaunchKernelGGL(cb_bwd_dwsa_partial_kernel, dim3(nt, nwc), dim3(256), 0, s, w.dpre, sin_, H, W, ksa, P, nwc,
-                       w.wpart);
-    if ((e = check_launch("cb_bwd_dwsa_partial"))) return e;
-    hipLaunchKernelGGL(cb_bwd_dwsa_final_kernel, dim3((unsigned)cdiv(nt, 128)), dim3(128), 0, s, w.wpart, nt, nwc, dwsa);
-    if ((e = check_launch("cb_bwd_dwsa_final"))) return e;
+    if ((e = sa_backward_launch(w.dpre, sin_, wsa, N, H, W, ksa, w.dsin, w.wpart, dwsa, s))) return e;
     const bool v4 = (C % 4 == 0) && (C / 4 <= 256) && (256 % (C / 4) == 0);
     if (fused)
         hipLaunchKernelGGL(cb_bwd_sums4_kernel<true>, dim3(N, nch), dim3(256), 0, s, dout, y, scale, shift, ca, sa, w.dsin,
@@ -888,7 +976,7 @@
         hipLaunchKernelGGL(cb_bwd_sums_kernel, dim3(N, nch), dim3(256), 0, s, dout, y, scale, shift, ca, sa, w.dsin,
                            sarg, HW, C, nch, w.parts);
     if ((e = check_launch("cb_bwd_sums"))) return e;
-    hipLaunchKernelGGL(cb_bwd_ca_kernel, dim3(N), dim3(256), (size_t)(4 * C + 2 * Cr) * sizeof(float), s, w.parts, nch,
+    hipLaunchKernelGGL(cb_bwd_ca_kernel, dim3(N), dim3(CA_THREADS), (size_t)(4 * C + 2 * Cr) * sizeof(float), s, w.parts, nch,
                        ymax, scale, shift, ca, w1, w2, HW, C, Cr, w.coef, w.dwpart);
     if ((e = check_launch("cb_bwd_ca"))) return e;
     hipLaunchKernelGGL(cb_bwd_dw_reduce_kernel, dim3((unsigned)cdiv(2LL * C * Cr, 256)), dim3(256), 0, s, w.dwpart, N,
diff --git a/ducosy-gan_amd/csrc/conv.hip b/ducosy-gan_amd/csrc/conv.hip
--- a/ducosy-gan_amd/csrc/conv.hip
+++ b/ducosy-gan_amd/csrc/conv.hip
@@ -1895,7 +1895,10 @@
 bool narrow_tiled_ok(const dcs_conv_desc& d, const float* src);
 int launch_narrow_rows_tiled(const dcs_conv_desc& d, const float* src, const float* wp, const float* bias,
                              const float* psc, const float* psh, float* out, hipStream_t s);
-bool narrow_small_ok(const dcs_conv_desc& d, const float* src);
+bool narrow_small_ok(const dcs_conv_desc& d, const float* src, const float* psc, const float* psh);
+int narrow_wgrad_small_blocks(const dcs_conv_desc& d);
+int launch_narrow_wgrad_small(const dcs_conv_desc& d, const float* dy, const float* src, const float* psc,
+                              const float* psh, float* part, hipStream_t s);
 int launch_narrow_rows_small(const dcs_conv_desc& d, const float* src, const float* wp, const float* bias,
                              const float* psc, const float* psh, float* out, hipStream_t s);
 bool narrow_wgrad_tiled_ok(const dcs_conv_desc& d, const float* src);
@@ -2868,7 +2871,7 @@
         if (M > Mmax) Mmax = M;
     }
     hipStream_t s = as_stream(stream);
-    if (narrow_small_ok(d, src)) return launch_narrow_rows_small(d, src, wpack, bias, psc, psh, out, s);
+    if (narrow_small_ok(d, src, psc, psh)) return launch_narrow_rows_small(d, src, wpack, bias, psc, psh, out, s);
     if (narrow_tiled_ok(d, src)) return launch_narrow_rows_tiled(d, src, wpack, bias, psc, psh, out, s);
     dim3 grid((unsigned)cdiv(Mmax, 256), ncls);
     const bool vec = vec_ok(dp, src);
@@ -2906,6 +2909,8 @@
     ClassGeom g = class_geom(*dp, 0);
     size_t naive = (size_t)ns * dp->Co * g.ntaps * dp->Cs * sizeof(float);
     size_t tiled = (size_t)narrow_wgrad_tiled_blocks(*dp) * g.ntaps * dp->Cs * sizeof(float);
+    size_t strip = (size_t)narrow_wgrad_small_blocks(*dp) * g.ntaps * dp->Cs * sizeof(float);
+    if (strip > tiled) tiled = strip;
     return naive > tiled ? naive : tiled;
 }
 
@@ -2931,6 +2936,13 @@
         hipLaunchKernelGGL(wgrad_reduce_kernel, dim3((unsigned)cdiv(Ktot, 256)), dim3(256), 0, s, w,
                            narrow_wgrad_tiled_blocks(d), 1, d.Cs, d.KH, d.KW, d.cw > 0 ? d.cw : d.Cs, dw);
         return check_launch("narrow_wgrad_tiled_reduce");
+    }
+    if (narrow_small_ok(d, x, psc, psh) && !x2) {
+        e = launch_narrow_wgrad_small(d, dy, x, psc, psh, w, s);
+        if (e) return e;
+        hipLaunchKernelGGL(wgrad_reduce_kernel, dim3((unsigned)cdiv(Ktot, 256)), dim3(256), 0, s, w,
+                           narrow_wgrad_small_blocks(d), 1, d.Cs, d.KH, d.KW, d.cw > 0 ? d.cw : d.Cs, dw);
+        return check_launch("narrow_wgrad_strip_reduce");
     }
     if (d.Co == 1) hipLaunchKernelGGL((conv_wgrad_narrow_kernel<1, false>), grid, dim3(256), 0, s, d, dy, x, x2, psc, psh, w, pps);
     else if (d.Co == 2) hipLaunchKernelGGL((conv_wgrad_narrow_kernel<2, false>), grid, dim3(256), 0, s, d, dy, x, x2, psc, psh, w, pps);
diff --git a/ducosy-gan_amd/csrc/conv_narrow.hip b/ducosy-gan_amd/csrc/conv_narrow.hip
--- a/ducosy-gan_amd/csrc/conv_narrow.hip
+++ b/ducosy-gan_amd/csrc/conv_narrow.hip
@@ -237,88 +237,217 @@
     }
 }
 
-template <int KH, int KW, int CPL>
-__global__ __launch_bounds__(256) void narrow_rows_small_kernel(const dcs_conv_desc d, const float* __restrict__ src,
+constexpr int NS_S = 8, NS_K = 4;
+
+template <int CPL>
+__device__ __forceinline__ void strip_pixel(const dcs_conv_desc& d, const float* __restrict__ sp, bool in,
+                                            const float4* sc, const float4* sh, float4* a) {
+#pragma unroll
+    for (int q = 0; q < CPL / 4; ++q) {
+        float4 v = *reinterpret_cast<const float4*>(sp + 4 * q);
+        if (d.pro_act != DCS_ACT_NONE) {
+            v.x = act_apply(fmaf(v.x, sc[q].x, sh[q].x), d.pro_act);
+            v.y = act_apply(fmaf(v.y, sc[q].y, sh[q].y), d.pro_act);
+            v.z = act_apply(fmaf(v.z, sc[q].z, sh[q].z), d.pro_act);
+            v.w = act_apply(fmaf(v.w, sc[q].w, sh[q].w), d.pro_act);
+        }
+        a[q] = in ? v : make_float4(0.f, 0.f, 0.f, 0.f);
+    }
+}
+
+template <int CPL>
+__global__ __launch_bounds__(256) void narrow_rows_strip_kernel(const dcs_conv_desc d, const float* __restrict__ src,
                                                                 const float* __restrict__ wp,
                                                                 const float* __restrict__ bias,
                                                                 const float* __restrict__ psc,
                                                                 const float* __restrict__ psh,
                                                                 float* __restrict__ out) {
     static_assert(CPL % 4 == 0, "float4 channel groups");
-    const int lane = threadIdx.x & 63;
+    constexpr int K = NS_K, Q4 = CPL / 4, CS = 64 * CPL;
+    __shared__ __attribute__((aligned(16))) float lw[K * K * CS];
+    const int lane = threadIdx.x & 63, wv = __builtin_amdgcn_readfirstlane(threadIdx.x >> 6);
+    for (int i = threadIdx.x; i < K * K * CS; i += 256) {
+        const int t = i / CS, c = i - t * CS;
+        lw[((t * Q4 + (c % CPL) / 4) * 64 + c / CPL) * 4 + (c & 3)] = wp[((long long)t * d.Cs + c) * d.ldb];
+    }
+    __syncthreads();
     const int c0 = lane * CPL;
-    float w[KH * KW][CPL];
-#pragma unroll
-    for (int t = 0; t < KH * KW; ++t)
-#pragma unroll
-        for (int j = 0; j < CPL; ++j) w[t][j] = wp[((long long)t * d.Cs + c0 + j) * d.ldb];
     const float b = bias ? bias[0] : 0.f;
-    const long long P = (long long)d.N * d.Ho * d.Wo;
-    const long long wave = ((long long)blockIdx.x * blockDim.x + threadIdx.x) >> 6;
-    const long long nwaves = ((long long)gridDim.x * blockDim.x) >> 6;
-    for (long long p = wave; p < P; p += nwaves) {
-        const int n = (int)(p / ((long long)d.Ho * d.Wo));
-        const int rem = (int)(p - (long long)n * d.Ho * d.Wo);
-        const int oy = rem / d.Wo, ox = rem - (rem / d.Wo) * d.Wo;
-        float sc[CPL], sh[CPL];
+    const int sx = (d.Wo + NS_S - 1) / NS_S;
+    const int nstrips = d.N * d.Ho * sx;
+    for (int st = blockIdx.x * 4 + wv; st < nstrips; st += gridDim.x * 4) {
+        const int n = st / (d.Ho * sx), rem = st - n * d.Ho * sx;
+        const int oy = rem / sx, ox0 = (rem - oy * sx) * NS_S;
+        float4 sc[Q4], sh[Q4];
         if (d.pro_act != DCS_ACT_NONE) {
 #pragma unroll
-            for (int j = 0; j < CPL; ++j) {
-                sc[j] = psc[(long long)n * d.Cs + c0 + j];
-                sh[j] = psh[(long long)n * d.Cs + c0 + j];
-            }
-        }
-        float acc = 0.f;
-#pragma unroll
-        for (int ty = 0; ty < KH; ++ty) {
-            const int iy = oy * d.stride + ty - d.pt;
+            for (int q = 0; q < Q4; ++q) {
+                sc[q] = *reinterpret_cast<const float4*>(psc + (long long)n * d.Cs + c0 + 4 * q);
+                sh[q] = *reinterpret_cast<const float4*>(psh + (long long)n * d.Cs + c0 + 4 * q);
+            }
+        }
+        float acc[NS_S];
+#pragma unroll
+        for (int o = 0; o < NS_S; ++o) acc[o] = 0.f;
+#pragma unroll
+        for (int ty = 0; ty < K; ++ty) {
+            const int iy = oy + ty - d.pt;
             if (iy < 0 || iy >= d.Hs) continue;
-#pragma unroll
-            for (int tx = 0; tx < KW; ++tx) {
-                const int ix = ox * d.stride + tx - d.pl;
-                if (ix < 0 || ix >= d.Ws) continue;
-                const float* sp = src + n * d.s_n + iy * d.s_h + ix * d.s_w + c0;
-#pragma unroll
-                for (int j4 = 0; j4 < CPL / 4; ++j4) {
-                    const float4 v4 = *reinterpret_cast<const float4*>(sp + 4 * j4);
-                    const float v[4] = {v4.x, v4.y, v4.z, v4.w};
-#pragma unroll
-                    for (int e = 0; e < 4; ++e) {
-                        const int j = 4 * j4 + e;
-                        const float a = d.pro_act != DCS_ACT_NONE ? act_apply(fmaf(v[e], sc[j], sh[j]), d.pro_act) : v[e];
-                        acc = fmaf(a, w[ty * KW + tx][j], acc);
+            float4 w[K][Q4];
+#pragma unroll
+            for (int tx = 0; tx < K; ++tx)
+#pragma unroll
+                for (int q = 0; q < Q4; ++q)
+                    w[tx][q] = *reinterpret_cast<const float4*>(lw + (((ty * K + tx) * Q4 + q) * 64 + lane) * 4);
+#pragma unroll
+            for (int i = 0; i < NS_S + K - 1; ++i) {
+                const int ix = ox0 + i - d.pl;
+                const bool in = ix >= 0 && ix < d.Ws;
+                float4 a[Q4];
+                strip_pixel<CPL>(d, src + n * d.s_n + iy * d.s_h + (in ? ix : 0) * d.s_w + c0, in, sc, sh, a);
+#pragma unroll
+                for (int q = 0; q < Q4; ++q)
+#pragma unroll
+                    for (int tx = 0; tx < K; ++tx) {
+                        const int o = i - tx;
+                        if (o >= 0 && o < NS_S) acc[o] = dot4(a[q], w[tx][q], acc[o]);
+                    }
+            }
+        }
+#pragma unroll
+        for (int o = 0; o < NS_S; ++o) {
+            float v = acc[o];
+#pragma unroll
+            for (int x = 32; x >= 1; x >>= 1) v += __shfl_xor(v, x, 64);
+            if (lane == 0 && ox0 + o < d.Wo) {
+                v += b;
+                if (d.epi_act != DCS_ACT_NONE) v = act_apply(v, d.epi_act);
+                out[((long long)n * d.Ho + oy) * d.Wo + ox0 + o] = v;
+            }
+        }
+    }
+}
+
+constexpr int NS_WGRAD_WAVES = 8;
+
+template <int CPL>
+__global__ __launch_bounds__(64 * NS_WGRAD_WAVES) void narrow_wgrad_strip_kernel(const dcs_conv_desc d,
+                                                                                 const float* __restrict__ dy,
+                                                                                 const float* __restrict__ src,
+                                                                                 const float* __restrict__ psc,
+                                                                                 const float* __restrict__ psh,
+                                                                                 float* __restrict__ part) {
+    static_assert(CPL % 4 == 0, "float4 channel groups");
+    constexpr int K = NS_K, Q4 = CPL / 4, CS = 64 * CPL, WV = NS_WGRAD_WAVES;
+    __shared__ __attribute__((aligned(16))) float red[K * K * CS];
+    const int lane = threadIdx.x & 63, wv = __builtin_amdgcn_readfirstlane(threadIdx.x >> 6);
+    const int c0 = lane * CPL;
+    float4 acc[K * K][Q4];
+#pragma unroll
+    for (int t = 0; t < K * K; ++t)
+#pragma unroll
+        for (int q = 0; q < Q4; ++q) acc[t][q] = make_float4(0.f, 0.f, 0.f, 0.f);
+    const int sx = (d.Ws + NS_S - 1) / NS_S;
+    const int nseg = d.N * d.Hs * sx;
+    for (int sg = blockIdx.x * WV + wv; sg < nseg; sg += gridDim.x * WV) {
+        const int n = sg / (d.Hs * sx), rem = sg - n * d.Hs * sx;
+        const int iy = rem / sx, ix0 = (rem - iy * sx) * NS_S;
+        float4 sc[Q4], sh[Q4];
+        if (d.pro_act != DCS_ACT_NONE) {
+#pragma unroll
+            for (int q = 0; q < Q4; ++q) {
+                sc[q] = *reinterpret_cast<const float4*>(psc + (long long)n * d.Cs + c0 + 4 * q);
+                sh[q] = *reinterpret_cast<const float4*>(psh + (long long)n * d.Cs + c0 + 4 * q);
+            }
+        }
+        const float* dyn = dy + (long long)n * d.Ho * d.Wo;
+#pragma unroll
+        for (int i = 0; i < NS_S; ++i) {
+            const int ix = ix0 + i;
+            const bool in = ix < d.Ws;
+            float4 a[Q4];
+            strip_pixel<CPL>(d, src + n * d.s_n + iy * d.s_h + (in ? ix : 0) * d.s_w + c0, in, sc, sh, a);
+#pragma unroll
+            for (int ty = 0; ty < K; ++ty) {
+                const int oy = iy + d.pt - ty;
+#pragma unroll
+                for (int tx = 0; tx < K; ++tx) {
+                    const int ox = ix + d.pl - tx;
+                    const bool ok = oy >= 0 && oy < d.Ho && ox >= 0 && ox < d.Wo;
+                    const float g = ok ? dyn[oy * d.Wo + ox] : 0.f;
+#pragma unroll
+                    for (int q = 0; q < Q4; ++q) {
+                        float4& r = acc[ty * K + tx][q];
+                        r.x = fmaf(g, a[q].x, r.x);
+                        r.y = fmaf(g, a[q].y, r.y);
+                        r.z = fmaf(g, a[q].z, r.z);
+                        r.w = fmaf(g, a[q].w, r.w);
                     }
                 }
             }
         }
-#pragma unroll
-        for (int o = 32; o >= 1; o >>= 1) acc += __shfl_xor(acc, o, 64);
-        if (lane == 0) {
-            float v = acc + b;
-            if (d.epi_act != DCS_ACT_NONE) v = act_apply(v, d.epi_act);
-            out[p] = v;
-        }
-    }
-}
-
-bool narrow_small_ok(const dcs_conv_desc& d, const float* src) {
-    return !d.parity && d.Co == 1 && d.up == 1 && d.pad_mode == DCS_PAD_ZERO && d.KH == 4 && d.KW == 4 &&
-           (d.Cs == 256 || d.Cs == 512) && d.s_c == 1 && d.csplit == d.Cs && d.s_w % 4 == 0 && d.s_h % 4 == 0 &&
-           d.s_n % 4 == 0 && (reinterpret_cast<uintptr_t>(src) & 15) == 0 && (long long)d.Ho * d.Wo <= 64 * 64;
+    }
+    for (int w = 0; w < WV; ++w) {
+        __syncthreads();
+        if (wv == w) {
+#pragma unroll
+            for (int t = 0; t < K * K; ++t)
+#pragma unroll
+                for (int q = 0; q < Q4; ++q) {
+                    float4* p = reinterpret_cast<float4*>(red + ((t * Q4 + q) * 64 + lane) * 4);
+                    float4 v = acc[t][q];
+                    if (w > 0) {
+                        const float4 u = *p;
+                        v.x += u.x; v.y += u.y; v.z += u.z; v.w += u.w;
+                    }
+                    *p = v;
+                }
+        }
+    }
+    __syncthreads();
+    for (int i = threadIdx.x; i < K * K * CS; i += 64 * WV) {
+        const int t = i / CS, c = i - t * CS;
+        part[(long long)blockIdx.x * (K * K * CS) + i] = red[((t * Q4 + (c % CPL) / 4) * 64 + c / CPL) * 4 + (c & 3)];
+    }
+}
+
+bool narrow_small_ok(const dcs_conv_desc& d, const float* src, const float* psc, const float* psh) {
+    const bool pro16 = d.pro_act == DCS_ACT_NONE ||
+                       ((reinterpret_cast<uintptr_t>(psc) | reinterpret_cast<uintptr_t>(psh)) & 15) == 0;
+    return !d.parity && d.Co == 1 && d.up == 1 && d.stride == 1 && d.pad_mode == DCS_PAD_ZERO && d.KH == 4 &&
+           d.KW == 4 && (d.Cs == 256 || d.Cs == 512) && d.s_c == 1 && d.csplit == d.Cs && d.s_w % 4 == 0 &&
+           d.s_h % 4 == 0 && d.s_n % 4 == 0 && (reinterpret_cast<uintptr_t>(src) & 15) == 0 && pro16 &&
+           (long long)d.Ho * d.Wo <= 64 * 64;
 }
 
 int launch_narrow_rows_small(const dcs_conv_desc& d, const float* src, const float* wp, const float* bias,
                              const float* psc, const float* psh, float* out, hipStream_t s) {
-    const long long P = (long long)d.N * d.Ho * d.Wo;
-    long long blocks = cdiv(P, 4);
-    if (blocks > 2048) blocks = 2048;
+    const long long strips = (long long)d.N * d.Ho * cdiv(d.Wo, NS_S);
+    long long blocks = cdiv(strips, 4);
+    if (blocks > 1024) blocks = 1024;
     if (d.Cs == 512)
-        hipLaunchKernelGGL((narrow_rows_small_kernel<4, 4, 8>), dim3((unsigned)blocks), dim3(256), 0, s, d, src, wp, bias,
-                           psc, psh, out);
+        hipLaunchKernelGGL((narrow_rows_strip_kernel<8>), dim3((unsigned)blocks), dim3(256), 0, s, d, src, wp, bias, psc,
+                           psh, out);
     else
-        hipLaunchKernelGGL((narrow_rows_small_kernel<4, 4, 4>), dim3((unsigned)blocks), dim3(256), 0, s, d, src, wp, bias,
-                           psc, psh, out);
-    return check_launch("narrow_rows_small");
+        hipLaunchKernelGGL((narrow_rows_strip_kernel<4>), dim3((unsigned)blocks), dim3(256), 0, s, d, src, wp, bias, psc,
+                           psh, out);
+    return check_launch("narrow_rows_strip");
+}
+
+int narrow_wgrad_small_blocks(const dcs_conv_desc& d) {
+    const long long segs = (long long)d.N * d.Hs * cdiv(d.Ws, NS_S);
+    const long long blocks = cdiv(segs, 2 * NS_WGRAD_WAVES);
+    return (int)(blocks > 256 ? 256 : blocks);
+}
+
+int launch_narrow_wgrad_small(const dcs_conv_desc& d, const float* dy, const float* src, const float* psc,
+                              const float* psh, float* part, hipStream_t s) {
+    const dim3 grid(narrow_wgrad_small_blocks(d)), block(64 * NS_WGRAD_WAVES);
+    if (d.Cs == 512)
+        hipLaunchKernelGGL((narrow_wgrad_strip_kernel<8>), grid, block, 0, s, d, dy, src, psc, psh, part);
+    else
+        hipLaunchKernelGGL((narrow_wgrad_strip_kernel<4>), grid, block, 0, s, d, dy, src, psc, psh, part);
+    return check_launch("narrow_wgrad_strip");
 }
 
 bool narrow_tiled_ok(const dcs_conv_desc& d, const float* src) {
diff --git a/ducosy-gan_amd/modules/hip/lib.py b/ducosy-gan_amd/modules/hip/lib.py
--- a/ducosy-gan_amd/modules/hip/lib.py
+++ b/ducosy-gan_amd/modules/hip/lib.py
@@ -128,6 +128,8 @@
     "dcs_conv_wgrad_narrow": (c_int, [DP, P, P, P, P, P, P, P, c_size_t, P]),
     "dcs_cbam_forward": (c_int, [P, P, P, P, P, P, P, P, c_int, c_int, c_int, c_int, c_int, c_int,
                                  P, P, P, P, P, P, P]),
+    "dcs_cbam_sa_backward_workspace_size": (c_size_t, [c_int, c_int, c_int, c_int]),
+    "dcs_cbam_sa_backward": (c_int, [P, P, P, c_int, c_int, c_int, c_int, P, P, P, c_size_t, P]),
     "dcs_cbam_backward_workspace_size": (c_size_t, [c_int, c_int, c_int, c_int, c_int, c_int]),
     "dcs_cbam_backward": (c_int, [P, P, P, P, P, P, P, P, P, P, P, P, P, c_int, c_int, c_int, c_int,
                                   c_int, c_int, P, P, P, P, P, c_size_t, P, P]),
diff --git a/ducosy-gan_amd/modules/hip/ops.py b/ducosy-gan_amd/modules/hip/ops.py
--- a/ducosy-gan_amd/modules/hip/ops.py
+++ b/ducosy-gan_amd/modules/hip/ops.py
@@ -471,6 +471,7 @@
         return self._attach_h3(out, w, 1) if (self.win and ci == self.cin) else out
 
     def _pack(self, w, kind, ci_count, K, ncols):
+        _check_dev(w)
         if kind in (0, 1) and ncols > 4 and self.kslice:
             kind |= lib.PACK_KSLICE
         if ncols <= 4:
@@ -964,6 +965,18 @@
     return out, (ca, sin_, sarg, sa)
 
 
+def cbam_sa_backward(dpre, sin_, wsa):
+    N, H, W = dpre.shape
+    ksa = wsa.shape[-1]
+    dsin = torch.empty(N, H * W, 2, device=dpre.device, dtype=torch.float32)
+    dwsa = torch.empty_like(wsa)
+    nb = lib.query("dcs_cbam_sa_backward_workspace_size", N, H, W, ksa)
+    ws = workspace(nb, dpre.device)
+    lib.call("dcs_cbam_sa_backward", _p(dpre), _p(sin_), _p(wsa), N, H, W, ksa, _p(dsin), _p(dwsa), _p(ws),
+             ws.numel(), _stream())
+    return dsin, dwsa
+
+
 def cbam_backward(dout, y, st: INStats, w1, w2, wsa, saved, out_dw=(None, None, None)):
     ca, sin_, sarg, sa = saved
     N, H, W, C = y.shape
diff --git a/include/ducosy_hip.h b/include/ducosy_hip.h
--- a/include/ducosy_hip.h
+++ b/include/ducosy_hip.h
@@ -227,6 +227,9 @@
                      int N, int H, int W, int C, int Cr, int ksa,
                      float* ca, float* sin_, int32_t* sarg, float* sa, float* out, float* rng,
                      void* stream);
+size_t dcs_cbam_sa_backward_workspace_size(int N, int H, int W, int ksa);
+int dcs_cbam_sa_backward(const float* dpre, const float* sin_, const float* wsa, int N, int H, int W,
+                         int ksa, float* dsin, float* dwsa, void* ws, size_t ws_bytes, void* stream);
 size_t dcs_cbam_backward_workspace_size(int N, int H, int W, int C, int Cr, int ksa);
 int dcs_cbam_backward(const float* dout, const float* y, const float* scale, const float* shift,
                       const float* ymax, const int32_t* yargmax, const float* w1, const float* w2,
```

Measured after the change: 39.47 img/s (median of 6 runs). About the same (+0.9%).
